# vocdoni/zk-franchise-proof-circuit

Measured on AMD Instinct MI355X. Metric: zkCensus proofs/sec (nLevels=160), higher is better.
Workload: dtype u256 (8 x u32 Montgomery, BN254 Fr/Fq)

## Files before the change

include/zkcensus.h:

```cpp
#ifndef ZKCENSUS_H
#define ZKCENSUS_H
#include <stddef.h>
#include <stdint.h>
#ifdef __cplusplus
extern "C" {
#endif

typedef struct zkc_ctx zkc_ctx;
typedef struct zkc_zkey zkc_zkey;

enum {
    ZKC_OK = 0,
    ZKC_ERR_GENERIC = 1,
    ZKC_ERR_SHORT_BUFFER = 2,
    ZKC_ERR_INVALID_WITNESS_LENGTH = 3,
    ZKC_ERR_BAD_ARG = 4,
    ZKC_ERR_FORMAT = 5,
    ZKC_ERR_HIP = 6,
    ZKC_ERR_WITNESS = 7
};
enum {
    ZKC_W_OK = 0, ZKC_W_ERR_WEIGHT = 1 , ZKC_W_ERR_SIK_ROOT = 2 ,
    ZKC_W_ERR_CENSUS_ROOT = 3 , ZKC_W_ERR_NULLIFIER = 4 , ZKC_W_ERR_LAST_SIBLING = 5 ,
    ZKC_W_ERR_INPUT_RANGE = 6 ,
    ZKC_W_ERR_SIK_LAST_SIBLING = 7
};
const char* zkc_witness_status_text(int nLevels, int32_t status);

int  zkc_ctx_create(int hip_device, zkc_ctx** out);
void zkc_ctx_destroy(zkc_ctx* ctx);
const char* zkc_last_error(const zkc_ctx* ctx);
void* zkc_ctx_stream(zkc_ctx* ctx);

int zkc_circuit_n_inputs(int nLevels);
int zkc_circuit_n_wires(int nLevels);
int zkc_circuit_nlevels_from_wasm(const void* wasm, size_t len, char sha256_hex[65]);
void zkc_sha256(const void* data, size_t len, uint8_t out[32]);

int zkc_witness(zkc_ctx* ctx, int nLevels, const void* inputs, int B, void* wtns, int32_t* status);
int zkc_inputs_from_json(const char* json, size_t len, int nLevels, void* out, char* err, size_t errlen);
int zkc_witness_dev(zkc_ctx* ctx, int nLevels, const void* d_inputs, int B, void* d_wtns, int32_t* d_status );

int  zkc_zkey_load(zkc_ctx* ctx, const void* zkey_bytes, size_t len, zkc_zkey** out);
void zkc_zkey_free(zkc_zkey* zk);
int  zkc_zkey_info(const zkc_zkey* zk, uint32_t* nVars, uint32_t* nPublic, uint32_t* domainSize);
int  zkc_zkey_pass_info(const zkc_zkey* zk, int* pass_size, int* lanes);
int  zkc_zkey_header_info(const void* zkey_bytes, size_t len, uint32_t* nVars, uint32_t* nPublic, uint32_t* domainSize);
int  zkc_zkey_sha256(const zkc_zkey* zk, uint8_t out[32]);
int  zkc_zkey_fingerprint(const void* zkey_bytes, size_t len, uint8_t out[32]);

void zkc_random_scalars(uint8_t* out, size_t n);
int zkc_prove(zkc_zkey* zk, const void* wtns, uint32_t nWitness, const uint8_t r[32], const uint8_t s[32],
              uint8_t proof[256], uint8_t* public_out);
int zkc_prove_dev(zkc_zkey* zk, const void* d_wtns, uint32_t nWitness, const uint8_t r[32], const uint8_t s[32],
                  uint8_t proof[256], uint8_t* public_out);

int zkc_prove_batch_dev(zkc_zkey* zk, const void* d_wtns, uint32_t nWitness, int B, const uint8_t* rs, uint8_t* proofs, uint8_t* publics);

int zkc_fullprove_batch_dev(zkc_zkey* zk, const void* d_inputs, int B, void* d_wtns, int32_t* d_status, const uint8_t* rs, uint8_t* proofs, uint8_t* publics);

int zkc_batch_begin(zkc_zkey* zk, int slot, const void* d_inputs, int B, void* d_wtns, int32_t* d_status, const uint8_t* rs);
int zkc_batch_finish(zkc_zkey* zk, int slot, uint8_t* proofs, uint8_t* publics);

typedef struct zkc_pool zkc_pool;
int  zkc_pool_create(const int* hip_devices, int n, zkc_pool** out);
void zkc_pool_destroy(zkc_pool* pool);
int  zkc_pool_size(const zkc_pool* pool);
zkc_ctx*  zkc_pool_ctx(zkc_pool* pool, int i);
zkc_zkey* zkc_pool_zkey(zkc_pool* pool, int i);
const char* zkc_pool_last_error(const zkc_pool* pool);
int  zkc_pool_zkey_load(zkc_pool* pool, const void* zkey_bytes, size_t len);
int  zkc_pool_fullprove_batch(zkc_pool* pool, const void* inputs, int B, const uint8_t* rs, uint8_t* proofs, uint8_t* publics, int32_t* status);

typedef struct zkc_service zkc_service;
typedef void (*zkc_done_fn)(void* user, int rc, int32_t witness_status, const char* error_text );
int  zkc_service_create(const int* hip_devices, int n, zkc_service** out);
void zkc_service_destroy(zkc_service* svc);
zkc_service* zkc_service_default(void);
const char* zkc_service_last_error(void);
int zkc_service_fullprove(zkc_service* svc, const void* zkey, size_t zkey_len, int nLevels, const void* inputs , const uint8_t* rs,
                          uint8_t proof[256], uint8_t* publics , int32_t* status, char* err, size_t errlen);
int zkc_service_prove(zkc_service* svc, const void* zkey, size_t zkey_len, const void* wtns , uint32_t nWitness, const uint8_t* rs,
                      uint8_t proof[256], uint8_t* publics, char* err, size_t errlen);
int zkc_service_fullprove_json(zkc_service* svc, const void* zkey, size_t zkey_len, const void* wasm, size_t wasm_len, const char* inputs_json, size_t inputs_len,
                               const uint8_t* rs, uint8_t proof[256], uint8_t* publics, int32_t* status, char* err, size_t errlen);
int zkc_service_submit_fullprove(zkc_service* svc, const void* zkey, size_t zkey_len, int nLevels, const void* inputs, const uint8_t* rs,
                                 uint8_t proof[256], uint8_t* publics, zkc_done_fn done, void* user);
int zkc_service_submit_prove(zkc_service* svc, const void* zkey, size_t zkey_len, const void* wtns, uint32_t nWitness, const uint8_t* rs,
                             uint8_t proof[256], uint8_t* publics, zkc_done_fn done, void* user);
int zkc_service_stats(zkc_service* svc, uint64_t out[8]);
int zkc_service_timing(zkc_service* svc, uint64_t out[8]);
int zkc_service_memory(zkc_service* svc, uint64_t out[8]);

int groth16_prover(const void* zkey_buffer, unsigned long zkey_size, const void* wtns_buffer, unsigned long wtns_size,
                   char* proof_buffer, unsigned long* proof_size, char* public_buffer, unsigned long* public_size,
                   char* error_msg, unsigned long error_msg_maxsize);

int groth16_fullprove(const void* zkey_buffer, unsigned long zkey_size, const void* wasm_buffer, unsigned long wasm_size, const char* inputs_json, unsigned long inputs_size,
                      char* proof_buffer, unsigned long* proof_size, char* public_buffer, unsigned long* public_size,
// ... 87 lines not shown
```

zk-franchise-proof-circuit_amd/__init__.py:

```python
import ctypes
from . import _native
from ._native import ZkcError
from .inputs import INPUT_KEYS, flatten_inputs, R_MOD

__all__ = ['Context', 'ProvingKey', 'DevicePool', 'ProvingService', 'groth16', 'ZkcError', 'INPUT_KEYS', 'flatten_inputs', 'R_MOD']


class Context:

    def __init__(self, device=0):
        self._lib = _native.load()
        h = ctypes.c_void_p()
        rc = self._lib.zkc_ctx_create(int(device), ctypes.byref(h))
        if rc != 0:
            raise ZkcError(rc, (self._lib.zkc_last_error(None) or b'').decode())
        self._h = h
        self.device = device
        self._keys = []

    def close(self):
        if getattr(self, '_h', None):
            for k in list(self._keys):
                k.close()
            self._lib.zkc_ctx_destroy(self._h)
            self._h = None

    def __del__(self):
        try:
            self.close()
        except Exception:
            pass

    def _check(self, rc, allow=()):
        if rc != 0 and rc not in allow:
            raise ZkcError(rc, (self._lib.zkc_last_error(self._h) or b'').decode())
        return rc

    @property
    def stream(self):
        return self._lib.zkc_ctx_stream(self._h)

    def n_wires(self, nLevels=160):
        return self._lib.zkc_circuit_n_wires(nLevels)

    def n_inputs(self, nLevels=160):
        return self._lib.zkc_circuit_n_inputs(nLevels)

    def witness(self, inputs, nLevels=160):
        flat = b''.join(x if isinstance(x, (bytes, bytearray)) else flatten_inputs(x, nLevels) for x in inputs)
        B = len(inputs)
        nw = self.n_wires(nLevels)
        out = ctypes.create_string_buffer(B * nw * 32)
        st = (ctypes.c_int32 * B)()
        self._check(self._lib.zkc_witness(self._h, nLevels, flat, B, out, st), allow=(7,))
        raw = out.raw
        return [raw[i * nw * 32:(i + 1) * nw * 32] for i in range(B)], list(st)

    def witness_dev(self, d_inputs_ptr, B, d_wtns_ptr, d_status_ptr, nLevels=160):
        self._check(self._lib.zkc_witness_dev(self._h, nLevels, d_inputs_ptr, B, d_wtns_ptr, d_status_ptr))


class ProvingKey:

    def __init__(self, ctx, zkey_bytes):
        self.ctx = ctx
        self._lib = ctx._lib
        h = ctypes.c_void_p()
        ctx._check(self._lib.zkc_zkey_load(ctx._h, zkey_bytes, len(zkey_bytes), ctypes.byref(h)))
        self._h = h
        ctx._keys.append(self)
        a, b, c = ctypes.c_uint32(), ctypes.c_uint32(), ctypes.c_uint32()
        self._lib.zkc_zkey_info(h, ctypes.byref(a), ctypes.byref(b), ctypes.byref(c))
        self.n_vars, self.n_public, self.domain_size = a.value, b.value, c.value
        ps, ln = ctypes.c_int(), ctypes.c_int()
        self._lib.zkc_zkey_pass_info(h, ctypes.byref(ps), ctypes.byref(ln))
        self.pass_size, self.lanes = ps.value, ln.value

    def close(self):
        if getattr(self, '_h', None):
            if getattr(self.ctx, '_h', None):
                self._lib.zkc_zkey_free(self._h)
            self._h = None
            if self in self.ctx._keys:
                self.ctx._keys.remove(self)

    def __del__(self):
        try:
            self.close()
        except Exception:
            pass

    @staticmethod
    def _scalar(x):
        return x if isinstance(x, (bytes, bytearray)) else int(x).to_bytes(32, 'little')

    def prove(self, wtns, r, s):
        proof = ctypes.create_string_buffer(256); pub = ctypes.create_string_buffer(32 * self.n_public)
        self.ctx._check(self._lib.zkc_prove(self._h, wtns, len(wtns) // 32, self._scalar(r), self._scalar(s), proof, pub))
        return proof.raw, pub.raw

    def prove_dev(self, d_wtns_ptr, r, s):
        proof = ctypes.create_string_buffer(256); pub = ctypes.create_string_buffer(32 * self.n_public)
        self.ctx._check(self._lib.zkc_prove_dev(self._h, d_wtns_ptr, self.n_vars, self._scalar(r), self._scalar(s), proof, pub))
        return proof.raw, pub.raw

    def prove_batch_dev(self, d_wtns_ptr, B, rs):
        proofs = ctypes.create_string_buffer(256 * B); pubs = ctypes.create_string_buffer(32 * self.n_public * B)
        self.ctx._check(self._lib.zkc_prove_batch_dev(self._h, d_wtns_ptr, self.n_vars, B, bytes(rs), proofs, pubs))
        return proofs.raw, pubs.raw

    def fullprove_batch_dev(self, d_inputs_ptr, B, d_wtns_ptr, d_status_ptr, rs):
        proofs = ctypes.create_string_buffer(256 * B); pubs = ctypes.create_string_buffer(32 * self.n_public * B)
        self.ctx._check(self._lib.zkc_fullprove_batch_dev(self._h, d_inputs_ptr, B, d_wtns_ptr, d_status_ptr, bytes(rs), proofs, pubs))
        return proofs.raw, pubs.raw

    def batch_begin(self, slot, d_inputs_ptr, B, d_wtns_ptr, d_status_ptr, rs):
        self.ctx._check(self._lib.zkc_batch_begin(self._h, slot, d_inputs_ptr, B, d_wtns_ptr, d_status_ptr, bytes(rs)))

    def batch_finish(self, slot, B):
        proofs = ctypes.create_string_buffer(256 * B); pubs = ctypes.create_string_buffer(32 * self.n_public * B)
        self.ctx._check(self._lib.zkc_batch_finish(self._h, slot, proofs, pubs))
        return proofs.raw, pubs.raw

    def debug_stage(self, d_wtns_ptr, stage):
        out = ctypes.create_string_buffer((96 if stage == 0 else 32) * self.domain_size)
        self.ctx._check(self._lib.zkc_debug_stage(self._h, d_wtns_ptr, stage, out))
        return out.raw

    def msm_debug(self, which, d_scalars_ptr, count):
# ... 114 lines not shown
```

zk-franchise-proof-circuit_amd/_native.py:

```python
import ctypes
import os

_HERE = os.path.dirname(os.path.abspath(__file__))
LIB_PATH = os.environ.get('ZKCENSUS_LIB') or os.path.join(_HERE, 'libzkcensus.so')
_lib = None


class ZkcError(RuntimeError):
    def __init__(self, code, msg):
        super().__init__('libzkcensus error %d: %s' % (code, msg))
        self.code = code


def load():
    global _lib
    if _lib is not None:
        return _lib
    if not os.path.exists(LIB_PATH):
        raise ImportError('libzkcensus.so is not built (run `python -c "import __graft_entry__ as g; g.build()"`); '
                          'there is no CPU fallback for the product path')
    try:
        import torch
    except ImportError:
        pass
    L = ctypes.CDLL(LIB_PATH)
    vp, i32p = ctypes.c_void_p, ctypes.POINTER(ctypes.c_int32)
    L.zkc_ctx_create.argtypes = [ctypes.c_int, ctypes.POINTER(vp)]
    L.zkc_ctx_destroy.argtypes = [vp]
    L.zkc_last_error.argtypes = [vp]; L.zkc_last_error.restype = ctypes.c_char_p
    L.zkc_ctx_stream.argtypes = [vp]; L.zkc_ctx_stream.restype = vp
    L.zkc_witness.argtypes = [vp, ctypes.c_int, vp, ctypes.c_int, vp, i32p]
    L.zkc_witness_dev.argtypes = [vp, ctypes.c_int, vp, ctypes.c_int, vp, vp]
    u8p, u32p = ctypes.c_char_p, ctypes.POINTER(ctypes.c_uint32)
    L.zkc_zkey_load.argtypes = [vp, ctypes.c_char_p, ctypes.c_size_t, ctypes.POINTER(vp)]
    L.zkc_zkey_free.argtypes = [vp]; L.zkc_zkey_free.restype = None
    L.zkc_zkey_info.argtypes = [vp, u32p, u32p, u32p]
    L.zkc_zkey_pass_info.argtypes = [vp, ctypes.POINTER(ctypes.c_int), ctypes.POINTER(ctypes.c_int)]
    L.zkc_witness_status_text.argtypes = [ctypes.c_int, ctypes.c_int32]; L.zkc_witness_status_text.restype = ctypes.c_char_p
    L.zkc_prove.argtypes = [vp, ctypes.c_char_p, ctypes.c_uint32, u8p, u8p, ctypes.c_char_p, ctypes.c_char_p]
    L.zkc_prove_dev.argtypes = [vp, vp, ctypes.c_uint32, u8p, u8p, ctypes.c_char_p, ctypes.c_char_p]
    L.zkc_prove_batch_dev.argtypes = [vp, vp, ctypes.c_uint32, ctypes.c_int, ctypes.c_char_p, ctypes.c_char_p, ctypes.c_char_p]
    L.zkc_fullprove_batch_dev.argtypes = [vp, vp, ctypes.c_int, vp, vp, ctypes.c_char_p, ctypes.c_char_p, ctypes.c_char_p]
    L.zkc_debug_stage.argtypes = [vp, vp, ctypes.c_int, ctypes.c_char_p]
    L.zkc_debug_early_retries.argtypes = []; L.zkc_debug_early_retries.restype = ctypes.c_ulonglong
    L.zkc_msm_debug.argtypes = [vp, ctypes.c_int, vp, ctypes.c_uint32, ctypes.c_char_p]
    L.zkc_debug_pairing_dev.argtypes = [vp, ctypes.c_char_p, ctypes.c_char_p, ctypes.c_char_p, ctypes.c_int, ctypes.c_char_p, ctypes.c_char_p, i32p, ctypes.POINTER(ctypes.c_int),
                                        ctypes.POINTER(ctypes.c_uint32), ctypes.c_size_t, ctypes.c_char_p]
    ulp = ctypes.POINTER(ctypes.c_ulong)
    L.groth16_prover.argtypes = [ctypes.c_char_p, ctypes.c_ulong, ctypes.c_char_p, ctypes.c_ulong, ctypes.c_char_p, ulp, ctypes.c_char_p, ulp, ctypes.c_char_p, ctypes.c_ulong]
    L.zkc_verify.argtypes = [ctypes.c_char_p, ctypes.c_char_p, ctypes.c_char_p]
    L.zkc_verify_bin.argtypes = [ctypes.c_char_p, ctypes.c_int, ctypes.c_char_p, ctypes.c_char_p]
    L.zkc_verify_batch.argtypes = [vp, ctypes.c_char_p, ctypes.c_int, ctypes.c_char_p, ctypes.c_char_p, ctypes.c_int, ctypes.c_char_p]
    L.zkc_verify_batch_each.argtypes = [vp, ctypes.c_char_p, ctypes.c_int, ctypes.c_char_p, ctypes.c_char_p, ctypes.c_int, ctypes.c_char_p, i32p]
    L.zkc_verify_each_stats.argtypes = [vp, ctypes.POINTER(ctypes.c_uint64)]
    L.zkc_verify_last_error.restype = ctypes.c_char_p
    L.zkc_proof_to_json.argtypes = [ctypes.c_char_p, ctypes.c_char_p, ctypes.c_int, ctypes.c_char_p, ulp, ctypes.c_char_p, ulp]
    L.zkc_proof_from_json.argtypes = [ctypes.c_char_p, ctypes.c_char_p, ctypes.c_char_p, ctypes.c_char_p, ctypes.POINTER(ctypes.c_int)]
    L.zkc_vkey_from_json.argtypes = [ctypes.c_char_p, ctypes.c_char_p, ulp, ctypes.POINTER(ctypes.c_int)]
    L.zkc_wtns_parse.argtypes = [ctypes.c_char_p, ctypes.c_ulong, ctypes.POINTER(ctypes.c_void_p), ctypes.POINTER(ctypes.c_uint32)]
    L.zkc_wtns_write.argtypes = [ctypes.c_char_p, ctypes.c_uint32, ctypes.c_char_p, ctypes.c_ulong]; L.zkc_wtns_write.restype = ctypes.c_ulong
    L.zkc_poseidon_batch.argtypes = [vp, ctypes.c_int, ctypes.c_char_p, ctypes.c_size_t, ctypes.c_char_p]
    L.zkc_smt_build.argtypes = [vp, ctypes.c_char_p, ctypes.c_char_p, ctypes.c_size_t, ctypes.c_int, ctypes.c_char_p, ctypes.c_char_p, i32p]
    L.zkc_census_inputs.argtypes = [vp, ctypes.c_size_t, ctypes.c_int, ctypes.c_char_p, ctypes.c_char_p, ctypes.c_char_p, ctypes.c_char_p, ctypes.c_char_p, ctypes.c_char_p, ctypes.c_char_p, vp, vp, ctypes.c_char_p]
    sz = ctypes.c_size_t
    L.zkc_tree_create.argtypes = [vp, ctypes.c_int, ctypes.POINTER(vp)]
    L.zkc_tree_free.argtypes = [vp]; L.zkc_tree_free.restype = None
    L.zkc_tree_add.argtypes = [vp, ctypes.c_char_p, ctypes.c_char_p, sz, i32p]
    L.zkc_tree_update.argtypes = [vp, ctypes.c_char_p, ctypes.c_char_p, sz, i32p]
    L.zkc_tree_delete.argtypes = [vp, ctypes.c_char_p, sz, i32p]
    L.zkc_tree_refs.argtypes = [vp, ctypes.POINTER(sz)]
    L.zkc_tree_snapshot.argtypes = [vp, ctypes.POINTER(vp)]
    L.zkc_tree_snapshot_count.argtypes = [vp, ctypes.POINTER(sz)]
    L.zkc_tree_gen_absence_proof.argtypes = [vp, ctypes.c_char_p, sz, ctypes.c_char_p, vp, i32p, vp, vp, i32p, i32p]
    L.zkc_tree_root.argtypes = [vp, ctypes.c_char_p]
    L.zkc_tree_size.argtypes = [vp, ctypes.POINTER(sz)]
    L.zkc_tree_get.argtypes = [vp, ctypes.c_char_p, sz, vp, i32p]
    L.zkc_tree_gen_proof.argtypes = [vp, ctypes.c_char_p, sz, ctypes.c_char_p, vp, i32p, i32p]
    L.zkc_tree_census_inputs.argtypes = [vp, vp, sz, ctypes.c_char_p, ctypes.c_char_p, ctypes.c_char_p, ctypes.c_char_p, ctypes.c_char_p, ctypes.c_char_p, vp, vp, ctypes.c_char_p, i32p]
    L.zkc_tree_stats.argtypes = [vp, ctypes.POINTER(ctypes.c_double)]
    L.zkc_smt_check_proofs.argtypes = [vp, ctypes.c_int, sz, ctypes.c_char_p, ctypes.c_char_p, ctypes.c_char_p, ctypes.c_char_p, ctypes.c_int, i32p]
    L.zkc_smt_check_absence.argtypes = [vp, ctypes.c_int, sz, ctypes.c_char_p, ctypes.c_char_p, ctypes.c_char_p, i32p, ctypes.c_char_p, ctypes.c_char_p, ctypes.c_int, i32p]
    L.zkc_smt_check_stats.argtypes = [vp, ctypes.POINTER(ctypes.c_double)]
    L.zkc_profile_enable.argtypes = [vp, ctypes.c_uint32]
    L.zkc_ntt_dev.argtypes = [vp, vp, vp, ctypes.c_int, ctypes.c_int, ctypes.c_int]
    L.zkc_g1_mul_batch_dev.argtypes = [vp, ctypes.c_char_p, vp, ctypes.c_uint32, vp]
    L.zkc_msm_g1_load_dev.argtypes = [vp, vp, ctypes.c_uint32, ctypes.POINTER(vp)]
    L.zkc_msm_g1_dev.argtypes = [vp, vp, ctypes.c_char_p]
    L.zkc_msm_g1_free.argtypes = [vp]; L.zkc_msm_g1_free.restype = None
    L.zkc_profile_read.argtypes = [vp, ctypes.c_int, ctypes.POINTER(ctypes.c_double), ctypes.POINTER(ctypes.c_uint64), ctypes.POINTER(ctypes.c_uint64)]
    L.zkc_setup_from_r1cs.argtypes = [ctypes.c_char_p, ctypes.c_uint64, ctypes.c_char_p, ctypes.c_char_p, ctypes.c_char_p, ctypes.c_size_t]
# ... 62 lines not shown
```

zk-franchise-proof-circuit_amd/csrc/zkc_api.hip:

```cpp
#include "zkc_internal.h"
#include "zkc_f29.h"
#include "zkc_kernels.h"
#include <array>
#include <cstring>
#include <ctime>
#include <map>
#include <mutex>
#include "../../include/zkc_poseidon_constants.inc"

using namespace zkc;

static constexpr int ZKC_WITNESS_WAVE_MAX_B = 128, ZKC_WITNESS_WAVE_MAX_B_ALONE = 1024;

static thread_local std::string g_create_err;

int zkc_fail(zkc_ctx* ctx, int code, const std::string& msg) {
    if (ctx) ctx->err = msg; else g_create_err = msg;
    return code;
}
hipError_t zkc_wait_event(hipEvent_t ev, unsigned spin_us) {
    if (sw::on<sw::ZKC_SPIN_WAIT>()) return hipEventSynchronize(ev);
    timespec t0; if (spin_us) clock_gettime(CLOCK_MONOTONIC, &t0);
    for (int i = 0;; i++) {
        const hipError_t e = hipEventQuery(ev);
// ... 5 lines not shown
}
hipError_t zkc_wait_stream(hipStream_t st, hipEvent_t scratch_ev) {
    const hipError_t e = hipEventRecord(scratch_ev, st);
    return e != hipSuccess ? e : zkc_wait_event(scratch_ev);
}
void zkc_ctx_lanes_destroy(zkc_ctx* ctx);
int zkc_ensure(zkc_ctx* ctx, void** p, size_t* cur, size_t need) {
    if (*cur >= need) return ZKC_OK;
    if (*p) { ZKC_HIP_CHECK(ctx, hipFree(*p)); *p = nullptr; *cur = 0; }
    ZKC_HIP_CHECK(ctx, hipMalloc(p, need));
    *cur = need;
    return ZKC_OK;
}

void zkc_verify_ws_trim(zkc_ctx* ctx, size_t keep_bytes) {
    size_t total = 0; for (size_t b : ctx->vws_sz) total += b;
    if (total <= keep_bytes && keep_bytes) return;
    for (int i = 0; i < zkc_ctx::VWS_N; i++) { if (ctx->vws[i]) (void)hipFree(ctx->vws[i]); ctx->vws[i] = nullptr; ctx->vws_sz[i] = 0; }
}

static hipEvent_t prof_event(zkc_ctx* ctx) {
    if (!ctx->prof.free_events.empty()) { hipEvent_t e = ctx->prof.free_events.back(); ctx->prof.free_events.pop_back(); return e; }
    hipEvent_t e = nullptr; (void)hipEventCreate(&e); return e;
}
zkc_prof_scope::zkc_prof_scope(zkc_ctx* c, int category, uint64_t alg_bytes, hipStream_t stream) : ctx(c), cat(category), st(stream ? stream : (c ? c->stream : nullptr)) {
    on = c && ((c->prof.mask >> category) & 1u);
    if (!on) return;
    a = prof_event(c); b = prof_event(c);
    c->prof.bytes[cat] += alg_bytes; c->prof.launches[cat] += 1;
    (void)hipEventRecord(a, st);
}
zkc_prof_scope::~zkc_prof_scope() {
    if (!on) return;
    (void)hipEventRecord(b, st);
    ctx->prof.pending.push_back({a, b, cat});
}
extern "C" int zkc_profile_enable(zkc_ctx* ctx, uint32_t mask) {
    if (!ctx) return ZKC_ERR_BAD_ARG;
    ZKC_LOCK(ctx);
    ZKC_HIP_CHECK(ctx, hipSetDevice(ctx->device));
    (void)hipStreamSynchronize(ctx->stream);
    for (auto& r : ctx->prof.pending) { ctx->prof.free_events.push_back(r.a); ctx->prof.free_events.push_back(r.b); }
    ctx->prof.pending.clear();
    for (int i = 0; i < ZKC_PROF_NCAT; i++) { ctx->prof.ms[i] = 0; ctx->prof.launches[i] = 0; ctx->prof.bytes[i] = 0; }
    if (!ctx->d_prof_entries && hipMalloc((void**)&ctx->d_prof_entries, 8) != hipSuccess) ctx->d_prof_entries = nullptr;
    if (ctx->d_prof_entries) (void)hipMemset(ctx->d_prof_entries, 0, 8);
    ctx->prof.mask = mask;
    return ZKC_OK;
}
extern "C" int zkc_profile_read(zkc_ctx* ctx, int cat, double* total_ms, uint64_t* launches, uint64_t* alg_bytes) {
    if (!ctx || cat < 0 || cat >= ZKC_PROF_NCAT) return ZKC_ERR_BAD_ARG;
    ZKC_LOCK(ctx);
    ZKC_HIP_CHECK(ctx, hipSetDevice(ctx->device));
    ZKC_HIP_CHECK(ctx, hipStreamSynchronize(ctx->stream)); ZKC_HIP_CHECK(ctx, hipStreamSynchronize(ctx->stream2)); ZKC_HIP_CHECK(ctx, hipStreamSynchronize(ctx->fin_stream));
    for (auto& r : ctx->prof.pending) {
        float ms = 0; (void)hipEventElapsedTime(&ms, r.a, r.b); ctx->prof.ms[r.cat] += ms;
        ctx->prof.free_events.push_back(r.a); ctx->prof.free_events.push_back(r.b);
    }
    ctx->prof.pending.clear();
    if (cat == ZKC_PROF_MSM_G1_STREAMED && ctx->d_prof_entries) {
        unsigned long long v = 0; (void)hipMemcpyAsync(&v, ctx->d_prof_entries, 8, hipMemcpyDeviceToHost, ctx->stream); (void)hipStreamSynchronize(ctx->stream); ctx->prof.launches[cat] = v;
    }
    if (total_ms) *total_ms = ctx->prof.ms[cat]; if (launches) *launches = ctx->prof.launches[cat]; if (alg_bytes) *alg_bytes = ctx->prof.bytes[cat];
    return ZKC_OK;
}

extern "C" int zkc_poseidon_batch(zkc_ctx* ctx, int n_inputs, const void* inputs, size_t B, void* out) {
    if (!ctx || !inputs || !out || n_inputs < 2 || n_inputs > 4 || B == 0) return zkc_fail(ctx, ZKC_ERR_BAD_ARG, "zkc_poseidon_batch: bad argument");
    ZKC_LOCK(ctx);
    ZKC_HIP_CHECK(ctx, hipSetDevice(ctx->device));
    int rc;
    if ((rc = zkc_ensure(ctx, &ctx->d_scratch_in, &ctx->scratch_in_sz, B * n_inputs * 32))) return rc;
    if ((rc = zkc_ensure(ctx, &ctx->d_scratch_out, &ctx->scratch_out_sz, B * 32))) return rc;
    ZKC_HIP_CHECK(ctx, hipMemcpyAsync(ctx->d_scratch_in, inputs, B * n_inputs * 32, hipMemcpyHostToDevice, ctx->stream));
    hipLaunchKernelGGL(zkc_poseidon_batch_kernel, dim3((unsigned)((B + 63) / 64)), dim3(64), 0, ctx->stream, ctx->ptab, (const uint32_t*)ctx->d_scratch_in,
                       (uint32_t*)ctx->d_scratch_out, n_inputs, B);
    ZKC_HIP_CHECK(ctx, hipGetLastError());
    ZKC_HIP_CHECK(ctx, hipMemcpyAsync(out, ctx->d_scratch_out, B * 32, hipMemcpyDeviceToHost, ctx->stream));
    ZKC_HIP_CHECK(ctx, hipStreamSynchronize(ctx->stream));
    return ZKC_OK;
}

__global__ void zkc_status_combine(const int32_t* __restrict__ s3, int32_t* __restrict__ s, int B) {
    int b = blockIdx.x * blockDim.x + threadIdx.x;
    if (b >= B) return;
    int m = s3[3 * b + 2], c = s3[3 * b + 0], k = s3[3 * b + 1], r = 0;
    if (m == ZKC_W_ERR_INPUT_RANGE) r = m;
    else if (m == ZKC_W_ERR_WEIGHT) r = m;
    else if (k) r = k; else if (c) r = c; else r = m;
    s[b] = r;
}

template <size_t N>
static void conv_consts(std::vector<Fr>& out, const unsigned long long (&src)[N][4]) {
    for (size_t i = 0; i < N; i++) {
        uint32_t s[8];
        for (int k = 0; k < 4; k++) { s[2 * k] = (uint32_t)src[i][k]; s[2 * k + 1] = (uint32_t)(src[i][k] >> 32); }
        out.push_back(fp_from_std<FrParams>(s));
    }
}


extern "C" int zkc_ctx_create(int device, zkc_ctx** out) {
    if (!out) return zkc_fail(nullptr, ZKC_ERR_BAD_ARG, "out == NULL");
    int ndev = 0;
    if (hipGetDeviceCount(&ndev) != hipSuccess || ndev <= 0)
        return zkc_fail(nullptr, ZKC_ERR_HIP, "no HIP device: libzkcensus has no CPU path (the CPU restatement lives in oracle/ and is test-only)");
    if (device < 0 || device >= ndev) return zkc_fail(nullptr, ZKC_ERR_BAD_ARG, "bad device ordinal");
    zkc_ctx* ctx = new zkc_ctx();
    ctx->device = device;
    auto fail = [&](hipError_t e, const char* what) { g_create_err = std::string(what) + ": " + hipGetErrorString(e); delete ctx; return (int)ZKC_ERR_HIP; };
    hipError_t e;
    if ((e = hipSetDevice(device)) != hipSuccess) return fail(e, "hipSetDevice");
    { if (sw::on<sw::ZKC_DEVICE_BLOCKING_SYNC>() && hipSetDeviceFlags(hipDeviceScheduleBlockingSync) != hipSuccess) (void)hipGetLastError(); }
    if ((e = hipStreamCreateWithFlags(&ctx->stream, hipStreamNonBlocking)) != hipSuccess) return fail(e, "hipStreamCreate");
    if ((e = hipStreamCreateWithFlags(&ctx->stream2, hipStreamNonBlocking)) != hipSuccess) return fail(e, "hipStreamCreate(2)");
    if ((e = hipStreamCreateWithFlags(&ctx->fin_stream, hipStreamNonBlocking)) != hipSuccess) return fail(e, "hipStreamCreate(fin)");
    std::vector<Fr> all; size_t off[12]; int k = 0;
    off[k++] = all.size(); conv_consts(all, ZKC_POSEIDON_C3); off[k++] = all.size(); conv_consts(all, ZKC_POSEIDON_S3);
    off[k++] = all.size(); conv_consts(all, ZKC_POSEIDON_M3); off[k++] = all.size(); conv_consts(all, ZKC_POSEIDON_P3);
    off[k++] = all.size(); conv_consts(all, ZKC_POSEIDON_C4); off[k++] = all.size(); conv_consts(all, ZKC_POSEIDON_S4);
    off[k++] = all.size(); conv_consts(all, ZKC_POSEIDON_M4); off[k++] = all.size(); conv_consts(all, ZKC_POSEIDON_P4);
    off[k++] = all.size(); conv_consts(all, ZKC_POSEIDON_C5); off[k++] = all.size(); conv_consts(all, ZKC_POSEIDON_S5);
    off[k++] = all.size(); conv_consts(all, ZKC_POSEIDON_M5); off[k++] = all.size(); conv_consts(all, ZKC_POSEIDON_P5);
    if ((e = hipMalloc(&ctx->d_ptab_mem, all.size() * sizeof(Fr))) != hipSuccess) return fail(e, "hipMalloc(poseidon)");
    if ((e = hipMemcpy(ctx->d_ptab_mem, all.data(), all.size() * sizeof(Fr), hipMemcpyHostToDevice)) != hipSuccess) return fail(e, "hipMemcpy(poseidon)");
    const Fr* base = (const Fr*)ctx->d_ptab_mem;
    {
        std::vector<uint32_t> l29(all.size() * 12, 0);
        for (size_t i = 0; i < all.size(); i++) { uint32_t t9[9]; f29_from_fp_shl5(t9, all[i].v); f29_mul<FrParams>(&l29[12 * i], t9, F29K<FrParams>::one.l); }
        if ((e = hipMalloc(&ctx->d_ptab29_mem, l29.size() * 4)) != hipSuccess) return fail(e, "hipMalloc(poseidon29)");
        if ((e = hipMemcpy(ctx->d_ptab29_mem, l29.data(), l29.size() * 4, hipMemcpyHostToDevice)) != hipSuccess) return fail(e, "hipMemcpy(poseidon29)");
        ctx->ptab.base = base; ctx->ptab.base29 = (const uint32_t*)ctx->d_ptab29_mem;
        std::vector<uint32_t> k29; size_t koff[2];
        for (int t = 3; t <= 4; t++) {
            koff[t - 3] = k29.size();
            const int RP = t == 3 ? 57 : 56; const size_t oC = off[(t - 3) * 4 + 0], oS = off[(t - 3) * 4 + 1];
            for (int r = 0; r < RP; r++) for (int k = 0; k < t; k++) {
                const size_t si = oS + (size_t)(2 * t - 1) * r + (k ? t + k - 1 : 0), ci = oC + 5 * t + r;
                const Fr prod = all[si] * all[ci];
                uint32_t t9[9], o9[12] = {0}; f29_from_fp_shl5(t9, prod.v); f29_mul<FrParams>(o9, t9, F29K<FrParams>::one.l); f29_reduce_small<FrParams>(o9);
                k29.insert(k29.end(), o9, o9 + 12);
            }
        }
        if ((e = hipMalloc(&ctx->d_pk29_mem, k29.size() * 4)) != hipSuccess) return fail(e, "hipMalloc(poseidon K29)");
        if ((e = hipMemcpy(ctx->d_pk29_mem, k29.data(), k29.size() * 4, hipMemcpyHostToDevice)) != hipSuccess) return fail(e, "hipMemcpy(poseidon K29)");
        for (int t = 3; t <= 4; t++) ctx->ptab.K29[t] = (const uint32_t*)ctx->d_pk29_mem + koff[t - 3];
    }
    for (int t = 3; t <= 5; t++) {
        ctx->ptab.C[t] = base + off[(t - 3) * 4 + 0]; ctx->ptab.S[t] = base + off[(t - 3) * 4 + 1];
        ctx->ptab.M[t] = base + off[(t - 3) * 4 + 2]; ctx->ptab.P[t] = base + off[(t - 3) * 4 + 3];
    }
    *out = ctx;
    return ZKC_OK;
}
extern "C" void zkc_ctx_destroy(zkc_ctx* ctx) {
    if (!ctx) return;
    (void)hipSetDevice(ctx->device);
    if (ctx->stream) (void)hipStreamSynchronize(ctx->stream);
    for (auto& r : ctx->prof.pending) { (void)hipEventDestroy(r.a); (void)hipEventDestroy(r.b); }
    for (auto e : ctx->prof.free_events) (void)hipEventDestroy(e);
    for (auto& kv : ctx->tmpl) (void)hipFree(kv.second);
    for (auto& kv : ctx->ntt_tw) { if (kv.second.fwd) (void)hipFree(kv.second.fwd); if (kv.second.inv) (void)hipFree(kv.second.inv); if (kv.second.ninv) (void)hipFree(kv.second.ninv); }
    if (ctx->d_ptab_mem) (void)hipFree(ctx->d_ptab_mem);
    if (ctx->d_ptab29_mem) (void)hipFree(ctx->d_ptab29_mem);
    if (ctx->d_pk29_mem) (void)hipFree(ctx->d_pk29_mem);
    if (ctx->d_scratch_in) (void)hipFree(ctx->d_scratch_in);
    if (ctx->d_scratch_out) (void)hipFree(ctx->d_scratch_out);
    if (ctx->d_status3) (void)hipFree(ctx->d_status3);
    if (ctx->d_status) (void)hipFree(ctx->d_status);
    if (ctx->d_prof_entries) (void)hipFree(ctx->d_prof_entries);
    for (int k = 0; k < 2; k++) {
        if (ctx->chk_h[k]) (void)hipHostFree(ctx->chk_h[k]);
        if (ctx->chk_d[k]) (void)hipFree(ctx->chk_d[k]);
        if (ctx->chk_ev[k]) (void)hipEventDestroy(ctx->chk_ev[k]);
    }
    zkc_verify_ws_trim(ctx, 0);
    if (ctx->ev_vws_up) (void)hipEventDestroy(ctx->ev_vws_up);
    if (ctx->ev_vws_lines) (void)hipEventDestroy(ctx->ev_vws_lines);
    for (auto& ls : ctx->lane_streams) for (hipStream_t q : {ls.st, ls.st2, ls.fin, ls.red}) if (q) (void)hipStreamSynchronize(q);
    zkc_ctx_lanes_destroy(ctx);
    if (ctx->ev_acc_chain) (void)hipEventDestroy(ctx->ev_acc_chain);
    if (ctx->stream2) (void)hipStreamDestroy(ctx->stream2);
    if (ctx->fin_stream) (void)hipStreamDestroy(ctx->fin_stream);
    if (ctx->stream) (void)hipStreamDestroy(ctx->stream);
    delete ctx;
}
int zkc_lane_streams(zkc_ctx* ctx, int l, bool with_red, zkc_ctx::LaneStreams* out) {
    if (!ctx || l < 0 || l >= 4 || !out) return ZKC_ERR_BAD_ARG;
    static std::mutex mu; static std::map<int, std::array<zkc_ctx::LaneStreams, 4>> by_device;
    std::lock_guard<std::mutex> g(mu);
    zkc_ctx::LaneStreams& ls = by_device[ctx->device][l];
    for (hipStream_t* q : {&ls.st, &ls.st2, &ls.fin}) if (!*q) ZKC_HIP_CHECK(ctx, hipStreamCreateWithFlags(q, hipStreamNonBlocking));
    if (with_red && !ls.red) ZKC_HIP_CHECK(ctx, hipStreamCreateWithFlags(&ls.red, hipStreamNonBlocking));
    ctx->lane_streams[l] = ls; *out = ls; return ZKC_OK;
}
extern "C" const char* zkc_last_error(const zkc_ctx* ctx) { return ctx ? ctx->err.c_str() : g_create_err.c_str(); }
extern "C" void* zkc_ctx_stream(zkc_ctx* ctx) { return ctx ? (void*)ctx->stream : nullptr; }
extern "C" int zkc_circuit_n_inputs(int nLevels) { return nLevels < 3 ? 0 : WitnessLayout::make(nLevels).nInputs; }
extern "C" int zkc_circuit_n_wires(int nLevels) { return nLevels < 3 ? 0 : WitnessLayout::make(nLevels).nWires; }

static int get_template(zkc_ctx* ctx, const WitnessLayout& L, uint32_t** out) {
    auto it = ctx->tmpl.find(L.nL);
    if (it != ctx->tmpl.end()) { *out = it->second; return ZKC_OK; }
    uint32_t *d_t = nullptr, *d_in = nullptr; int32_t* d_st = nullptr;
    const int rc = [&]() -> int {
        ZKC_HIP_CHECK(ctx, hipMalloc(&d_t, (size_t)L.nWires * 32));
        ZKC_HIP_CHECK(ctx, hipMalloc(&d_in, (size_t)L.nInputs * 32));
        ZKC_HIP_CHECK(ctx, hipMalloc(&d_st, 3 * sizeof(int32_t)));
        ZKC_HIP_CHECK(ctx, hipMemsetAsync(d_t, 0, (size_t)L.nWires * 32, ctx->stream));
        ZKC_HIP_CHECK(ctx, hipMemsetAsync(d_in, 0, (size_t)L.nInputs * 32, ctx->stream));
        hipLaunchKernelGGL(zkc_witness_chains_wave, dim3(3), dim3(64), 0, ctx->stream, L, ctx->ptab, d_in, d_t, d_st, 1, 1);
        hipLaunchKernelGGL(zkc_witness_tostd, dim3((L.nWires + 255) / 256), dim3(256), 0, ctx->stream, d_t, (size_t)L.nWires);
        ZKC_HIP_CHECK(ctx, hipGetLastError());
        ZKC_HIP_CHECK(ctx, hipStreamSynchronize(ctx->stream));
        return ZKC_OK;
    }();
    if (d_in) (void)hipFree(d_in);
    if (d_st) (void)hipFree(d_st);
    if (rc) { if (d_t) (void)hipFree(d_t); return rc; }
    ctx->tmpl[L.nL] = d_t; *out = d_t;
    return ZKC_OK;
}

uint32_t* zkc_get_template(zkc_ctx* ctx, int nLevels) {
    uint32_t* t = nullptr; WitnessLayout L = WitnessLayout::make(nLevels);
    return get_template(ctx, L, &t) == ZKC_OK ? t : nullptr;
}

static int witness_dev3(zkc_ctx* ctx, const WitnessLayout& L, const void* d_inputs, int B, void* d_wtns, int32_t* d_status3, bool alone, hipStream_t st = nullptr) {
    if (!st) st = ctx->stream;
    uint32_t* tmpl; int rc = get_template(ctx, L, &tmpl); if (rc) return rc;
    const size_t total = (size_t)L.nWires * 2 * (size_t)B;
    int fill_blocks = (int)std::min<size_t>((total + 255) / 256, 256 * 16);
    zkc_prof_scope _ps(ctx, ZKC_PROF_WITNESS, (uint64_t)B * ((uint64_t)L.nWires + L.nInputs) * 32, st);
    hipLaunchKernelGGL(zkc_witness_fill, dim3(fill_blocks), dim3(256), 0, st, (const uint4*)tmpl, (uint4*)d_wtns, L.nWires, B);
    ZKC_HIP_CHECK(ctx, hipGetLastError());
    if (B <= (alone ? ZKC_WITNESS_WAVE_MAX_B_ALONE : ZKC_WITNESS_WAVE_MAX_B))
        hipLaunchKernelGGL(zkc_witness_chains_wave, dim3(3 * B), dim3(64), 0, st, L, ctx->ptab, (const uint32_t*)d_inputs, (uint32_t*)d_wtns, d_status3, B, 0);
    else
        hipLaunchKernelGGL(zkc_witness_chains, dim3((3 * B + 63) / 64), dim3(64), 0, st, L, ctx->ptab, (const uint32_t*)d_inputs, (uint32_t*)d_wtns, d_status3, B, 0);
    {
        const size_t nw = (size_t)L.nWires * (size_t)B;
        hipLaunchKernelGGL(zkc_witness_tostd, dim3((unsigned)std::min<size_t>((nw + 255) / 256, 256 * 64)), dim3(256), 0, st, (uint32_t*)d_wtns, nw);
    }
    ZKC_HIP_CHECK(ctx, hipGetLastError());
// ... 43 lines not shown
```

zk-franchise-proof-circuit_amd/csrc/zkc_internal.h:

```cpp
#pragma once
#include <hip/hip_runtime.h>
#include <string>
#include <vector>
#include <map>
#include <mutex>
#include "../../include/zkcensus.h"
#include "zkc_device.h"
#include "zkc_switches.h"

#define ZKC_LOCK(ctx) std::lock_guard<std::recursive_mutex> _zkc_guard((ctx)->mu)
#define ZKC_HIP_CHECK(ctx, call)                                                                            \
    do { hipError_t _e = (call); if (_e != hipSuccess) {                                                     \
        return zkc_fail((ctx), ZKC_ERR_HIP, std::string(#call) + ": " + hipGetErrorString(_e)); } } while (0)

enum { ZKC_PROF_WITNESS = 0, ZKC_PROF_MATVEC = 1, ZKC_PROF_NTT = 2, ZKC_PROF_MSM_SORT = 3, ZKC_PROF_MSM_ACC_G1 = 4, ZKC_PROF_MSM_ACC_G2 = 5,
       ZKC_PROF_MSM_REDUCE = 6, ZKC_PROF_MSM_G1_STREAMED = 7 , ZKC_PROF_NCAT = 8 };
struct zkc_prof {
    uint32_t mask = 0;
    struct Rec { hipEvent_t a, b; int cat; };
    std::vector<Rec> pending; std::vector<hipEvent_t> free_events;
    double ms[ZKC_PROF_NCAT] = {0}; uint64_t launches[ZKC_PROF_NCAT] = {0}; uint64_t bytes[ZKC_PROF_NCAT] = {0};
};
struct zkc_ctx {
    std::recursive_mutex mu;
    int device = 0;
    hipStream_t stream = nullptr;
    hipStream_t stream2 = nullptr;
    hipStream_t fin_stream = nullptr;
    struct LaneStreams { hipStream_t st = nullptr, st2 = nullptr, fin = nullptr, red = nullptr; } lane_streams[4];
    struct zkc_lane* lanes = nullptr;
    hipEvent_t ev_acc_chain = nullptr; bool acc_chain_armed = false;
    std::string err;
    zkc::PoseidonTable ptab{};
    void* d_ptab_mem = nullptr;
    void* d_ptab29_mem = nullptr;
    void* d_pk29_mem = nullptr;
    std::map<int, uint32_t*> tmpl;
    struct TwiddleSet { uint32_t *fwd = nullptr, *inv = nullptr; void* ninv = nullptr; };
    std::map<int, TwiddleSet> ntt_tw;
    void* d_scratch_in = nullptr; size_t scratch_in_sz = 0;
    void* d_scratch_out = nullptr; size_t scratch_out_sz = 0;
    int32_t* d_status3 = nullptr; size_t status3_n = 0;
    int32_t* d_status = nullptr; size_t status_n = 0;
    enum { VWS_PTS = 0, VWS_RHO, VWS_IDX, VWS_GS, VWS_FOLD_TMP, VWS_FOLD_OUT, VWS_Q, VWS_LINES, VWS_TREE_A, VWS_TREE_B, VWS_BAD,
           VWS_FLAGS, VWS_SUM_TREE, VWS_TREE_ALL, VWS_NODES , VWS_N };
    void* vws[VWS_N] = {nullptr}; size_t vws_sz[VWS_N] = {0};
    uint64_t each_stats[4] = {0, 0, 0, 0};
    hipEvent_t ev_vws_up = nullptr, ev_vws_lines = nullptr;
    void* chk_h[2] = {nullptr, nullptr}; void* chk_d[2] = {nullptr, nullptr}; size_t chk_sz = 0; hipEvent_t chk_ev[2] = {nullptr, nullptr};
    double chk_ms[3] = {0, 0, 0};
    double r1cs_ms[3] = {0, 0, 0};
    zkc_prof prof;
    unsigned long long* d_prof_entries = nullptr;
};

int zkc_fail(zkc_ctx* ctx, int code, const std::string& msg);
hipError_t zkc_wait_event(hipEvent_t ev, unsigned spin_us = 0);
hipError_t zkc_wait_stream(hipStream_t st, hipEvent_t scratch_ev);
int zkc_ensure(zkc_ctx* ctx, void** p, size_t* cur, size_t need);
inline int zkc_vws(zkc_ctx* ctx, int which, size_t need, void** out) { const int rc = zkc_ensure(ctx, &ctx->vws[which], &ctx->vws_sz[which], need); *out = ctx->vws[which]; return rc; }
void zkc_verify_ws_trim(zkc_ctx* ctx, size_t keep_bytes);
struct zkc_prof_scope {
    zkc_ctx* ctx; int cat; hipEvent_t a = nullptr, b = nullptr; bool on; hipStream_t st;
    zkc_prof_scope(zkc_ctx* c, int category, uint64_t alg_bytes, hipStream_t stream = nullptr);
    ~zkc_prof_scope();
};
```

zk-franchise-proof-circuit_amd/csrc/zkc_pairing_dev.hip:

```cpp
#include <algorithm>
#include <cstdio>
#include <cstdlib>
#include <ctime>
#include <vector>
#include "zkc_prover.h"
#include "zkc_pairing.h"
#include "zkc_pairing_dev.h"

namespace zkc {
using namespace zkc::pairing;

struct MillerConsts { Fq2 twist_b, psi_x, psi_y, psi2_x, psi2_y; Fq half; uint64_t pos, neg; uint64_t t_lo, t_hi; };

__device__ __forceinline__ void store_line(Fq2* __restrict__ lines, uint32_t N, uint32_t step, uint32_t i, const Fq2 l[3]) {
    Fq2* o = lines + ((size_t)step * N + i) * 3; o[0] = l[0]; o[1] = l[1]; o[2] = l[2];
}
__device__ __forceinline__ bool g2_member(const G2Affine& q, const MillerConsts& C) {
    bool ok = fp_sqr(q.y) == fp_sqr(q.x) * q.x + C.twist_b;
    if (ok) {
        G2XYZZ acc = G2XYZZ::from_affine(q);
        for (int b = 125; b >= 0; b--) { acc = xyzz_dbl(acc); if (((b < 64 ? C.t_lo >> b : C.t_hi >> (b - 64)) & 1)) acc = xyzz_add_affine(acc, q); }
        ok = !acc.is_inf() && acc.X == conj2(q.x) * C.psi_x * acc.ZZ && acc.Y == conj2(q.y) * C.psi_y * acc.ZZZ;
    }
    return ok;
// ... 32 lines not shown
        if ((C.pos >> b) & 1) { line_add(R, q.x, q.y, l); store_line(lines, N, step++, i, l); }
        else if ((C.neg >> b) & 1) { line_add(R, q.x, nqy, l); store_line(lines, N, step++, i, l); }
    }
    line_add(R, conj2(q.x) * C.psi_x, conj2(q.y) * C.psi_y, l); store_line(lines, N, step++, i, l);
    line_add(R, q.x * C.psi2_x, fp_neg(q.y * C.psi2_y), l); store_line(lines, N, step++, i, l);
}
__device__ __forceinline__ void line_at(const Fq2* __restrict__ raw, const G1XYZZ& p, Fq2 out[3]) {
    if (p.is_inf()) { out[0] = Fq2::one(); out[1] = out[2] = Fq2::zero(); return; }
    out[0] = scale2(raw[0], fp_neg(p.Y * p.ZZ)); out[1] = scale2(raw[1], p.X * p.ZZZ); out[2] = scale2(raw[2], p.ZZ * p.ZZZ);
}
__global__ void __launch_bounds__(64)
zkc_line_pairs(const Fq2* __restrict__ lines, const G1XYZZ* __restrict__ P, uint32_t N, uint32_t nlines, Fq12* __restrict__ out) {
    const uint32_t half = (N + 1) / 2, gid = blockIdx.x * blockDim.x + threadIdx.x;
    if (gid >= nlines * half) return;
    const uint32_t s = gid / half, t = gid - s * half;
    const Fq2* a = lines + ((size_t)s * N + 2 * t) * 3;
    Fq2 l0[3], l1[3];
    line_at(a, P[2 * t], l0);
    if (2 * t + 1 < N) { line_at(a + 3, P[2 * t + 1], l1); out[(size_t)s * half + t] = mul_034_by_034(l0, l1); }
    else out[(size_t)s * half + t] = dense_of_034(l0);
}
__global__ void __launch_bounds__(64)
zkc_fq12_tree(const Fq12* __restrict__ in, uint32_t n, uint32_t nlines, Fq12* __restrict__ out) {
    const uint32_t half = (n + 1) / 2, gid = blockIdx.x * blockDim.x + threadIdx.x;
    if (gid >= nlines * half) return;
    const uint32_t s = gid / half, t = gid - s * half;
    const Fq12* a = in + (size_t)s * n + 2 * t;
    out[(size_t)s * half + t] = (2 * t + 1 < n) ? a[0] * a[1] : a[0];
}
__global__ void __launch_bounds__(64)
zkc_g1_sum_tree(const G1XYZZ* __restrict__ in, uint32_t n, G1XYZZ* __restrict__ out) {
    const uint32_t t = blockIdx.x * blockDim.x + threadIdx.x;
    if (t >= (n + 1) / 2) return;
    out[t] = (2 * t + 1 < n) ? xyzz_add(in[2 * t], in[2 * t + 1]) : in[2 * t];
}
__global__ void __launch_bounds__(64)
zkc_fq12_node(const Fq12* __restrict__ level, uint32_t m, uint32_t t, uint32_t nlines, Fq12* __restrict__ out) {
    const uint32_t s = blockIdx.x * blockDim.x + threadIdx.x;
    if (s < nlines && t < m) out[s] = level[(size_t)s * m + t];
}

static MillerConsts miller_consts() {
    const Consts& K = consts(); const AteLoop& L = ate_loop();
    MillerConsts C; C.twist_b = K.twist_b; C.psi_x = K.psi_x; C.psi_y = K.psi_y; C.psi2_x = K.psi2_x; C.psi2_y = K.psi2_y; C.half = K.half; C.pos = C.neg = 0;
    for (int b = 0; b < 64; b++) { if (L.digit[b] > 0) C.pos |= 1ull << b; else if (L.digit[b] < 0) C.neg |= 1ull << b; }
    C.t_lo = 0xf83e9682e87cfd46ull; C.t_hi = 0x6f4d8248eeb859fbull;
    return C;
}
static int dev_fail(zkc_ctx* ctx, hipError_t e, const char* what) { ctx->err = std::string(what) + ": " + hipGetErrorString(e); (void)hipGetLastError(); return ZKC_ERR_HIP; }

uint32_t verify_chunk() { return (uint32_t)sw::value<sw::ZKC_VERIFY_CHUNK>(16384); }
static uint32_t n_lines(const MillerConsts& C) { return 66 + (uint32_t)__builtin_popcountll(C.pos | C.neg); }
uint32_t verify_n_lines() { return n_lines(miller_consts()); }
void miller_join(zkc_ctx* ctx) { (void)hipStreamSynchronize(ctx->stream2); (void)hipStreamSynchronize(ctx->fin_stream); }

int miller_membership_begin(zkc_ctx* ctx, const G2Affine* h_Q, uint32_t N) {
    const MillerConsts C = miller_consts();
    const uint32_t cap = std::min(N, verify_chunk());
    void* q; int rc;
    if ((rc = zkc_vws(ctx, zkc_ctx::VWS_Q, (size_t)N * sizeof(G2Affine), &q))) return rc;
    G2Affine* d_Q = (G2Affine*)q;
    if ((rc = zkc_vws(ctx, zkc_ctx::VWS_BAD, sizeof(int), &q))) return rc;
    int* d_bad = (int*)q;
    if ((rc = zkc_vws(ctx, zkc_ctx::VWS_LINES, (size_t)n_lines(C) * cap * 3 * sizeof(Fq2), &q))) return rc;
    Fq2* d_lines = (Fq2*)q;
    hipError_t e;
    if (!ctx->ev_vws_up && (e = hipEventCreateWithFlags(&ctx->ev_vws_up, hipEventDisableTiming)) != hipSuccess) return dev_fail(ctx, e, "miller_membership_begin: hipEventCreate");
    if (!ctx->ev_vws_lines && (e = hipEventCreateWithFlags(&ctx->ev_vws_lines, hipEventDisableTiming)) != hipSuccess) return dev_fail(ctx, e, "miller_membership_begin: hipEventCreate");
    if ((e = hipMemcpyAsync(d_Q, h_Q, (size_t)N * sizeof(G2Affine), hipMemcpyHostToDevice, ctx->stream2)) != hipSuccess ||
        (e = hipMemsetAsync(d_bad, 0, sizeof(int), ctx->stream2)) != hipSuccess ||
        (e = hipEventRecord(ctx->ev_vws_up, ctx->stream2)) != hipSuccess ||
        (e = hipStreamWaitEvent(ctx->fin_stream, ctx->ev_vws_up, 0)) != hipSuccess ||
        (e = hipStreamWaitEvent(ctx->stream, ctx->ev_vws_up, 0)) != hipSuccess) { miller_join(ctx); return dev_fail(ctx, e, "miller_membership_begin: upload"); }
    hipLaunchKernelGGL(zkc_g2_membership, dim3((N + 63) / 64), dim3(64), 0, ctx->stream2, d_Q, N, C, d_bad);
    hipLaunchKernelGGL(zkc_miller_lines, dim3((cap + 63) / 64), dim3(64), 0, ctx->fin_stream, d_Q, cap, C, d_lines);
    if ((e = hipGetLastError()) != hipSuccess || (e = hipEventRecord(ctx->ev_vws_lines, ctx->fin_stream)) != hipSuccess) { miller_join(ctx); return dev_fail(ctx, e, "miller_membership_begin: launch"); }
    return ZKC_OK;
}
int miller_product_dev(zkc_ctx* ctx, const G1XYZZ* d_P, uint32_t N, Fq12* product, int* bad, std::vector<Fq12>* tops) {
    const MillerConsts C = miller_consts();
    const uint32_t nlines = n_lines(C), CHUNK = verify_chunk();
    const uint32_t cap = std::min(N, CHUNK), hcap = (cap + 1) / 2;
    const bool vtrace = sw::on<sw::ZKC_VERIFY_TRACE>();
    auto vnow = [] { timespec ts; clock_gettime(CLOCK_MONOTONIC, &ts); return ts.tv_sec * 1e3 + ts.tv_nsec * 1e-6; };
    const double mt0 = vnow(); double mt_chunks = 0;
    std::vector<Fq12> step(nlines), acc(nlines, one12());
    const int rc = [&]() -> int {
        const G2Affine* d_Q = (const G2Affine*)ctx->vws[zkc_ctx::VWS_Q];
        Fq2* d_lines = (Fq2*)ctx->vws[zkc_ctx::VWS_LINES];
        Fq12 *d_a, *d_b; void* q; int r;
        if ((r = zkc_vws(ctx, zkc_ctx::VWS_TREE_A, (size_t)nlines * hcap * sizeof(Fq12), &q))) return r; d_a = (Fq12*)q;
        if ((r = zkc_vws(ctx, zkc_ctx::VWS_TREE_B, (size_t)nlines * ((hcap + 1) / 2) * sizeof(Fq12), &q))) return r; d_b = (Fq12*)q;
        hipError_t e;
        for (uint32_t lo = 0; lo < N; lo += CHUNK) {
            const uint32_t n = std::min(CHUNK, N - lo);
            if ((e = hipStreamWaitEvent(ctx->stream, ctx->ev_vws_lines, 0)) != hipSuccess) return dev_fail(ctx, e, "miller_product_dev: event");
            uint32_t m = (n + 1) / 2;
            hipLaunchKernelGGL(zkc_line_pairs, dim3((nlines * m + 63) / 64), dim3(64), 0, ctx->stream, d_lines, d_P + lo, n, nlines, d_a);
            if (lo + CHUNK < N) {
                const uint32_t lo2 = lo + CHUNK, n2 = std::min(CHUNK, N - lo2);
                if ((e = hipEventRecord(ctx->ev_vws_up, ctx->stream)) != hipSuccess || (e = hipStreamWaitEvent(ctx->fin_stream, ctx->ev_vws_up, 0)) != hipSuccess) return dev_fail(ctx, e, "miller_product_dev: event");
                hipLaunchKernelGGL(zkc_miller_lines, dim3((n2 + 63) / 64), dim3(64), 0, ctx->fin_stream, d_Q + lo2, n2, C, d_lines);
                if ((e = hipEventRecord(ctx->ev_vws_lines, ctx->fin_stream)) != hipSuccess) return dev_fail(ctx, e, "miller_product_dev: event");
            }
            Fq12 *src = d_a, *dst = d_b;
            while (m > 1) {
                const uint32_t h = (m + 1) / 2;
                hipLaunchKernelGGL(zkc_fq12_tree, dim3((nlines * h + 63) / 64), dim3(64), 0, ctx->stream, src, m, nlines, dst);
                std::swap(src, dst); m = h;
            }
            if ((e = hipGetLastError()) != hipSuccess) return dev_fail(ctx, e, "miller_product_dev: launch");
            if ((e = hipMemcpyAsync(step.data(), src, (size_t)nlines * sizeof(Fq12), hipMemcpyDeviceToHost, ctx->stream)) != hipSuccess ||
// ... 93 lines not shown
```

zk-franchise-proof-circuit_amd/csrc/zkc_prove.hip:

```cpp
#include "zkc_prover.h"
#include "zkc_fixedbase.h"
#include "zkc_hostparse.h"
#include "zkc_kernels.h"
#include <cstring>
#include <ctime>
#include <cstdio>
#include <algorithm>
#include <atomic>

using namespace zkc;

static void matvec_launch(zkc_zkey* zk, zkc_lane& L, const uint32_t* d_wtns0, int nb, hipStream_t mv) {
    const uint32_t n = zk->n, nv = zk->nVars;
    const bool units = zk->n_unit_coeffs > 0 && nv <= 3 * (size_t)n && sw::on<sw::ZKC_MATVEC_UNITS>();
    if (units) hipLaunchKernelGGL(zkc_wtns_mont, dim3((nv + 255) / 256, nb), dim3(256), 0, mv, (const Fr*)d_wtns0, (size_t)nv, L.d_t, 3 * (size_t)n, nv);
    hipLaunchKernelGGL(zkc_matvec_jds, dim3((2 * n + 63 * zk->nlong + 255) / 256, nb), dim3(256), 0, mv, zk->d_perm, zk->d_rowlen, zk->d_jdptr, zk->d_col, zk->d_val,
                       (const Fr*)d_wtns0, (size_t)nv, L.d_abc, (int)n, zk->nlong, units ? (const Fr*)L.d_t : (const Fr*)nullptr, 3 * (size_t)n);
    hipLaunchKernelGGL(zkc_pointwise_mul, dim3((n + 255) / 256, nb), dim3(256), 0, mv, L.d_abc, (int)n);
}
static constexpr uint32_t MATVEC_LONG = 16;

namespace {
uint32_t rd32(const uint8_t* p) { uint32_t v; memcpy(&v, p, 4); return v; }
uint64_t rd64(const uint8_t* p) { uint64_t v; memcpy(&v, p, 8); return v; }
G1Affine rd_g1(const uint8_t* p) { G1Affine a; memcpy(a.x.v, p, 32); memcpy(a.y.v, p + 32, 32); return a; }
G2Affine rd_g2(const uint8_t* p) { G2Affine a; memcpy(a.x.c0.v, p, 32); memcpy(a.x.c1.v, p + 32, 32); memcpy(a.y.c0.v, p + 64, 32); memcpy(a.y.c1.v, p + 96, 32); return a; }
Fr fr_root_of_unity(int logn) {
    uint32_t e[8]; for (int i = 0; i < 8; i++) e[i] = FrParams::p[i]; e[0] -= 1;
    for (int i = 0; i < 8; i++) e[i] = (e[i] >> 28) | (i < 7 ? e[i + 1] << 4 : 0);
    Fr g = fp_from_u32<FrParams>(5), w = Fr::one();
    for (int i = 255; i >= 0; i--) { w = w * w; if ((e[i >> 5] >> (i & 31)) & 1) w = w * g; }
    for (int i = 28; i > logn; i--) w = w * w;
    return w;
}
template <class T> int dmalloc(zkc_ctx* ctx, T** p, size_t count) { ZKC_HIP_CHECK(ctx, hipMalloc((void**)p, count * sizeof(T))); return ZKC_OK; }
void g1_to_std(uint8_t* out, const G1Affine& a) { uint32_t s[8]; fp_to_std<FqParams>(s, a.x); memcpy(out, s, 32); fp_to_std<FqParams>(s, a.y); memcpy(out + 32, s, 32); }
void g2_to_std(uint8_t* out, const G2Affine& a) {
    uint32_t s[8]; fp_to_std<FqParams>(s, a.x.c0); memcpy(out, s, 32); fp_to_std<FqParams>(s, a.x.c1); memcpy(out + 32, s, 32);
    fp_to_std<FqParams>(s, a.y.c0); memcpy(out + 64, s, 32); fp_to_std<FqParams>(s, a.y.c1); memcpy(out + 96, s, 32);
}
}

uint32_t* zkc_get_template(zkc_ctx* ctx, int nLevels);
int zkc_lane_streams(zkc_ctx* ctx, int l, bool with_red, zkc_ctx::LaneStreams* out);

extern "C" __global__ void __launch_bounds__(64)
zkc_fold_check(WitnessLayout L, const uint32_t* __restrict__ wtns, const uint32_t* __restrict__ tmpl, uint32_t* __restrict__ flags, int B) {
    const int n = L.n, g = blockIdx.x, tree = blockIdx.y, b = blockIdx.z;
    const int blk = tree == 0 ? L.off_census : L.off_sikver;
    int start, end;
    if (g < n - 1) {
        const int nctrl = (g == n - 3) + (g > 0 && g < n - 2) + 1;
        start = blk + L.lvl_off(g) + nctrl; end = blk + (g + 1 < n - 1 ? L.lvl_off(g + 1) : L.lvl_off(n - 1));
    } else { start = blk + L.off_n2bold; end = start + 253 + 127 + 133; }
    const uint4* w = reinterpret_cast<const uint4*>(wtns + (size_t)b * L.nWires * 8) + 2 * (size_t)start;
    const uint4* t = reinterpret_cast<const uint4*>(tmpl) + 2 * (size_t)start;
    uint32_t diff = 0;
    for (int i = threadIdx.x; i < 2 * (end - start); i += 64) { uint4 x = w[i], y = t[i]; diff |= (x.x ^ y.x) | (x.y ^ y.y) | (x.z ^ y.z) | (x.w ^ y.w); }
    const unsigned long long any = __ballot(diff != 0);
    if (threadIdx.x == 0) flags[((size_t)b * 2 + tree) * n + g] = any ? 1u : 0u;
}

extern "C" __global__ void __launch_bounds__(64)
zkc_input_depths(const uint32_t* __restrict__ inputs, int nInputs, int n, uint32_t* __restrict__ out) {
    const int b = blockIdx.x, tree = blockIdx.y;
    const uint32_t* sib = inputs + ((size_t)b * nInputs + 12 + (size_t)tree * n) * 8;
    int d = 0;
    for (int i = threadIdx.x; i < n; i += 64) {
        const uint4* q = reinterpret_cast<const uint4*>(sib + 8 * (size_t)i); const uint4 x = q[0], y = q[1];
        if (x.x | x.y | x.z | x.w | y.x | y.y | y.z | y.w) d = i + 1;
    }
    for (int m = 32; m >= 1; m >>= 1) { const int o = __shfl_xor(d, m, 64); d = o > d ? o : d; }
    if (threadIdx.x == 0) out[2 * b + tree] = (uint32_t)d;
}

extern "C" void zkc_zkey_free(zkc_zkey* zk) {
    if (!zk) return;
    ZKC_LOCK(zk->ctx);
    (void)hipSetDevice(zk->ctx->device);
    (void)hipStreamSynchronize(zk->ctx->stream);
    void* ptrs[] = {zk->d_perm, zk->d_rowlen, zk->d_jdptr, zk->d_col, zk->d_val, zk->d_tw_fwd, zk->d_tw_inv, zk->d_tw_fwd29, zk->d_tw_inv29, zk->d_coset, zk->d_coset_br, zk->d_g1, zk->d_g2, zk->d_g2_29, zk->d_g2_29_lone, zk->d_g2_29_deep,
                    zk->d_tblDelta1, zk->d_tblAlpha1, zk->d_tblBeta1, zk->d_tblDelta2, zk->d_fb4, zk->d_fb4g2, zk->d_depths};
    for (void* p : ptrs) if (p) (void)hipFree(p);
    for (auto& kv : zk->fold.vmaps) if (kv.second.d) (void)hipFree(kv.second.d);
    for (void* q : {(void*)zk->fold.d_foldA, (void*)zk->fold.d_foldB1, (void*)zk->fold.d_foldC, (void*)zk->fold.d_foldB2}) if (q) (void)hipFree(q);
    if (zk->h_depths) (void)hipHostFree(zk->h_depths);
    for (auto& c : zk->call) { for (void* q : {(void*)c.d_rs, (void*)c.d_proofs, (void*)c.d_flags, (void*)c.d_status3}) if (q) (void)hipFree(q); if (c.h_flags) (void)hipHostFree(c.h_flags); if (c.h_out) (void)hipHostFree(c.h_out); if (c.h_rs) (void)hipHostFree(c.h_rs); if (c.h_xyzz) (void)hipHostFree(c.h_xyzz); if (c.h_early) (void)hipHostFree(c.h_early); if (c.d_xyzz) (void)hipFree(c.d_xyzz); for (hipEvent_t e : c.ev_done) if (e) (void)hipEventDestroy(e); for (hipEvent_t e : c.ev_chunk) (void)hipEventDestroy(e); }
    if (zk->ctx->lanes) for (int l = 0; l < zk->nlanes; l++) for (hipStream_t q : {zk->ctx->lanes[l].st, zk->ctx->lanes[l].st2, zk->ctx->lanes[l].fin, zk->ctx->lanes[l].red}) if (q) (void)hipStreamSynchronize(q);
    delete zk;
}

static size_t dev_free_bytes() { size_t f = 0, t = 0; if (hipMemGetInfo(&f, &t) != hipSuccess) { (void)hipGetLastError(); return 0; } return f; }
static int fold_prepare(zkc_zkey* zk);
static int fb4_prepare(zkc_zkey* zk);
struct LaneNeed { size_t abc, p, fin, bs, e1, b1, e2, b2; int j1, j2; };
static LaneNeed lane_need(const zkc_zkey* zk, int inflight) {
    const uint32_t n = zk->n, nv = zk->nVars; const int NWS = msm_nw(zk->c_sec), NWB = msm_nw(zk->c_h);
    const size_t per_proof_entries = (size_t)NWS * 3 * nv + (size_t)NWB * n;
    const size_t per_proof_buckets = 3 * (size_t)msm_half(std::max(zk->c_sec, zk->c_deep)) + msm_half(zk->c_h);
    LaneNeed nd; nd.abc = 3 * (size_t)n * inflight; nd.p = 8 * (size_t)n * inflight; nd.fin = finalize_scratch_bytes(inflight); nd.bs = 2 * 2 * 8 * (size_t)nv;
    nd.e1 = per_proof_entries * inflight; nd.b1 = per_proof_buckets * inflight; nd.j1 = 4 * inflight;
    nd.e2 = (size_t)NWS * nv * inflight; nd.b2 = (size_t)msm_half(std::max(zk->c_sec, zk->c_deep)) * inflight; nd.j2 = inflight;
    return nd;
}
static bool lane_holds(const zkc_lane& L, const LaneNeed& nd) {
    return L.cap_abc >= nd.abc && L.cap_p >= nd.p && L.cap_fin >= nd.fin && L.cap_bs >= nd.bs && L.w1.max_entries >= nd.e1 && L.w1.max_buckets >= nd.b1 && L.w1.max_jobs >= nd.j1 &&
           L.w2.max_entries >= nd.e2 && L.w2.max_buckets >= nd.b2 && L.w2.max_jobs >= nd.j2;
}
static void lane_release(zkc_lane& L) {
    for (void** q : {(void**)&L.d_abc, (void**)&L.d_t, (void**)&L.d_p, &L.d_fin, (void**)&L.d_bs}) if (*q) { (void)hipFree(*q); *q = nullptr; }
    msm_work_free(L.w1); msm_work_free(L.w2);
    L.cap_abc = L.cap_p = L.cap_fin = L.cap_bs = 0; L.bytes = 0;
}
static zkc_lane* ctx_lanes(zkc_ctx* ctx) { if (!ctx->lanes) ctx->lanes = new zkc_lane[MAX_LANES]; return ctx->lanes; }
static size_t ctx_work_bytes(const zkc_ctx* ctx) { size_t t = 0; if (ctx->lanes) for (int l = 0; l < MAX_LANES; l++) t += ctx->lanes[l].bytes; return t; }
void zkc_ctx_lanes_destroy(zkc_ctx* ctx) {
    if (!ctx->lanes) return;
    for (int l = 0; l < MAX_LANES; l++) {
        zkc_lane& L = ctx->lanes[l];
        lane_release(L);
        for (hipEvent_t e : {L.ev_msm, L.ev_msm2, L.ev_sorted, L.ev_ntt, L.ev_mv, L.ev_acc, L.ev_fin[0], L.ev_fin[1], L.ev_red}) if (e) (void)hipEventDestroy(e);
    }
    delete[] ctx->lanes; ctx->lanes = nullptr;
}
static int lane_init(zkc_ctx* ctx, int l) {
    zkc_lane& L = ctx_lanes(ctx)[l];
    if (L.made) return ZKC_OK;
    zkc_ctx::LaneStreams ls; int rc = zkc_lane_streams(ctx, l, sw::on<sw::ZKC_REDUCE_STREAM>(), &ls); if (rc) return rc;
    L.st = ls.st; L.st2 = ls.st2; L.fin = ls.fin; L.red = ls.red;
    for (hipEvent_t* e : {&L.ev_msm, &L.ev_msm2, &L.ev_sorted, &L.ev_ntt, &L.ev_mv, &L.ev_acc, &L.ev_fin[0], &L.ev_fin[1], &L.ev_red}) if (!*e) ZKC_HIP_CHECK(ctx, hipEventCreateWithFlags(e, hipEventDisableTiming));
    L.made = true; return ZKC_OK;
}
struct LaneSt { hipStream_t st, st2, fin, red; };
static LaneSt lane_st(const zkc_zkey* zk, const zkc_lane& L) { hipStream_t c = zk->ctx->stream; return zk->serial_streams ? LaneSt{c, c, c, c} : LaneSt{L.st, L.st2, L.fin, L.red}; }
static int lane_ensure(zkc_zkey* zk, int l, int inflight) {
    zkc_ctx* ctx = zk->ctx; int rc;
    if ((rc = lane_init(ctx, l))) return rc;
    zkc_lane& L = ctx->lanes[l];
    inflight = std::max(1, std::min(inflight, zk->max_inflight));
    if (lane_holds(L, lane_need(zk, inflight))) return ZKC_OK;
    inflight = std::min(inflight <= 4 ? 4 : zk->max_inflight, zk->max_inflight);
    LaneNeed nd = lane_need(zk, inflight);
    nd.abc = std::max(nd.abc, L.cap_abc); nd.p = std::max(nd.p, L.cap_p); nd.fin = std::max(nd.fin, L.cap_fin); nd.bs = std::max(nd.bs, L.cap_bs);
    nd.e1 = std::max(nd.e1, L.w1.max_entries); nd.b1 = std::max(nd.b1, L.w1.max_buckets); nd.j1 = std::max(nd.j1, L.w1.max_jobs);
    nd.e2 = std::max(nd.e2, L.w2.max_entries); nd.b2 = std::max(nd.b2, L.w2.max_buckets); nd.j2 = std::max(nd.j2, L.w2.max_jobs);
    for (hipStream_t q : {L.st, L.st2, L.fin, L.red}) if (q) ZKC_HIP_CHECK(ctx, hipStreamSynchronize(q));
    ZKC_HIP_CHECK(ctx, hipStreamSynchronize(ctx->stream));
    lane_release(L);
    const size_t free_before = dev_free_bytes();
    const auto fail_at = sw::given<sw::ZKC_TEST_FAIL_ALLOC>();
    rc = (fail_at && inflight >= *fail_at) ? zkc_fail(ctx, ZKC_ERR_HIP, "lanes_ensure: allocation failure injected by ZKC_TEST_FAIL_ALLOC") : ZKC_OK;
    if (!rc) rc = dmalloc(ctx, &L.d_abc, nd.abc);
    if (!rc) rc = dmalloc(ctx, &L.d_t, nd.abc);
    if (!rc) rc = dmalloc(ctx, &L.d_p, nd.p);
    if (!rc && hipMalloc(&L.d_fin, nd.fin) != hipSuccess) rc = zkc_fail(ctx, ZKC_ERR_HIP, "lanes_ensure: hipMalloc failed (blinding scratch)");
    if (!rc) rc = dmalloc(ctx, &L.d_bs, nd.bs);
    if (!rc) rc = msm_work_alloc(ctx, L.w1, nd.e1, nd.b1, nd.j1, false);
    if (!rc) rc = msm_work_alloc(ctx, L.w2, nd.e2, nd.b2, nd.j2, true);
    if (rc) { (void)hipGetLastError(); lane_release(L); return rc; }
    L.cap_abc = nd.abc; L.cap_p = nd.p; L.cap_fin = nd.fin; L.cap_bs = nd.bs;
    { const size_t f = dev_free_bytes(); L.bytes = free_before > f ? free_before - f : 0; }
    return ZKC_OK;
}
static int lanes_ensure(zkc_zkey* zk, int inflight, int first = 0, int count = -1) {
    if (count < 0) count = zk->nlanes - first;
    for (int l = first; l < first + count && l < zk->nlanes; l++) { const int rc = lane_ensure(zk, l, inflight); if (rc) return rc; }
    return ZKC_OK;
}
extern "C" int zkc_zkey_load(zkc_ctx* ctx, const void* zkey_bytes, size_t len, zkc_zkey** out) { return zkc::zkey_load_opts(ctx, zkey_bytes, len, 0, 0, out); }
size_t zkc::zkey_device_bytes(const zkc_zkey* zk, size_t* tables, size_t* work) {
    if (!zk) return 0;
    const size_t w = ctx_work_bytes(zk->ctx);
    if (tables) *tables = zk->bytes_tables; if (work) *work = w;
    return zk->bytes_tables + w;
}
int zkc::zkey_load_opts(zkc_ctx* ctx, const void* zkey_bytes, size_t len, int opt_lanes, int opt_inflight, zkc_zkey** out) {
    if (!ctx || !zkey_bytes || !out) return zkc_fail(ctx, ZKC_ERR_BAD_ARG, "zkc_zkey_load: bad argument");
    ZKC_LOCK(ctx);
    ZKC_HIP_CHECK(ctx, hipSetDevice(ctx->device));
    const size_t free_at_entry = dev_free_bytes(), work_at_entry = ctx_work_bytes(ctx);
    const uint8_t* buf = (const uint8_t*)zkey_bytes;
    parse::BinSections bs; parse::ZkeyHeader zh; std::string perr;
    if (!parse::binfile_sections(buf, len, "zkey", 1, bs, perr) || !parse::zkey_check(bs, zh, perr)) return zkc_fail(ctx, ZKC_ERR_FORMAT, perr);
    const uint8_t* const* sec = bs.sec;
    const uint8_t* h = sec[2];
    zkc_zkey* zk = new zkc_zkey(); zk->ctx = ctx;
    zk->nVars = zh.nVars; zk->nPub = zh.nPub; zk->n = zh.n; zk->logn = zh.logn; zk->nCoeffs = zh.nCoeffs;
    parse::sha256(buf, len, zk->sha256); parse::zkey_fingerprint(buf, len, bs, zk->fingerprint);
    const uint32_t n = zk->n, nv = zk->nVars, np = zk->nPub, nc = nv - np - 1;
    zk->alpha1 = rd_g1(h + 84); zk->beta1 = rd_g1(h + 148); zk->beta2 = rd_g2(h + 212); zk->gamma2 = rd_g2(h + 340);
// ... 71 lines not shown
      zk->c_deep = (zk->nLevels >= 0 && (nv >= (1u << 16) || dt == 2) && zk->c_sec < cd && dt != 0) ? cd : 0; }
    zk->c_h = std::max(zk->c_h, std::max(zk->c_sec, zk->c_deep));
    const int NWB = msm_nw(zk->c_h);
    zk->offA = 0; zk->offB1 = NWS * nv; zk->offC = 2 * NWS * nv; zk->offH = 2 * NWS * nv + NWS * nc;
    const int NWD = zk->c_deep ? msm_nw(zk->c_deep) : 0;
    zk->offA_deep = zk->offH + NWB * n; zk->offB1_deep = zk->offA_deep + NWD * nv; zk->offC_deep = zk->offB1_deep + NWD * nv;
    const size_t g1_points = (size_t)NWS * (2 * (size_t)nv + nc) + (size_t)NWB * n + (size_t)NWD * (2 * (size_t)nv + nc);
    if (g1_points >= (1ull << 31)) return bail(zkc_fail(ctx, ZKC_ERR_FORMAT, "zkey too large for 31-bit point indices"));
    if ((rc = dmalloc(ctx, &zk->d_g1, g1_points)) || (rc = dmalloc(ctx, &zk->d_g2, (size_t)NWS * nv))) return bail(rc);
    ZKC_UP(zk->d_g1 + zk->offA, sec[5], 64ull * nv); ZKC_UP(zk->d_g1 + zk->offB1, sec[6], 64ull * nv);
    ZKC_UP(zk->d_g1 + zk->offC, sec[8], 64ull * nc); ZKC_UP(zk->d_g1 + zk->offH, sec[9], 64ull * n);
    ZKC_UP(zk->d_g2, sec[7], 128ull * nv);
    if ((rc = msm_precompute_g1(ctx, nv, zk->d_g1 + zk->offA, zk->c_sec)) || (rc = msm_precompute_g1(ctx, nv, zk->d_g1 + zk->offB1, zk->c_sec)) ||
        (rc = msm_precompute_g1(ctx, nc, zk->d_g1 + zk->offC, zk->c_sec)) || (rc = msm_precompute_g1(ctx, n, zk->d_g1 + zk->offH, zk->c_h)) ||
        (rc = msm_precompute_g2(ctx, nv, zk->d_g2, zk->c_sec))) return bail(rc);
    if ((rc = dmalloc(ctx, &zk->d_g2_29, 60 * (size_t)NWS * nv)) || (rc = msm_g2_table29(ctx, zk->d_g2, zk->d_g2_29, (size_t)NWS * nv))) return bail(rc);
    if (zk->c_deep) {
        ZKC_UP(zk->d_g1 + zk->offA_deep, sec[5], 64ull * nv); ZKC_UP(zk->d_g1 + zk->offB1_deep, sec[6], 64ull * nv); ZKC_UP(zk->d_g1 + zk->offC_deep, sec[8], 64ull * nc);
        if ((rc = msm_precompute_g1(ctx, nv, zk->d_g1 + zk->offA_deep, zk->c_deep)) || (rc = msm_precompute_g1(ctx, nv, zk->d_g1 + zk->offB1_deep, zk->c_deep)) ||
            (rc = msm_precompute_g1(ctx, nc, zk->d_g1 + zk->offC_deep, zk->c_deep))) return bail(rc);
        G2Affine* tmp = nullptr;
        if ((rc = dmalloc(ctx, &tmp, (size_t)NWD * nv))) return bail(rc);
        hipError_t e2 = hipMemcpyAsync(tmp, zk->d_g2, 128ull * nv, hipMemcpyDeviceToDevice, ctx->stream);
        if (e2 == hipSuccess) rc = msm_precompute_g2(ctx, nv, tmp, zk->c_deep);
        if (e2 == hipSuccess && !rc) rc = dmalloc(ctx, &zk->d_g2_29_deep, 60 * (size_t)NWD * nv);
        if (e2 == hipSuccess && !rc) rc = msm_g2_table29(ctx, tmp, zk->d_g2_29_deep, (size_t)NWD * nv);
        if (e2 == hipSuccess && !rc) e2 = hipStreamSynchronize(ctx->stream);
        (void)hipFree(tmp);
        if (rc) return bail(rc);
        if (e2 != hipSuccess) return bail(zkc_fail(ctx, ZKC_ERR_HIP, std::string("second section tables: ") + hipGetErrorString(e2)));
    }
    {
        if (sw::on<sw::ZKC_G2_LONE_TABLE>() && (zk->nLevels >= 0 || nv < (1u << 16))) {
            constexpr int NWL = msm_nw(MSM_C_G2_LONE);
            G2Affine* tmp = nullptr;
            if ((rc = dmalloc(ctx, &tmp, (size_t)NWL * nv))) return bail(rc);
            hipError_t e2 = hipMemcpyAsync(tmp, zk->d_g2, 128ull * nv, hipMemcpyDeviceToDevice, ctx->stream);
            if (e2 == hipSuccess) rc = msm_precompute_g2(ctx, nv, tmp, MSM_C_G2_LONE);
            if (e2 == hipSuccess && !rc) rc = dmalloc(ctx, &zk->d_g2_29_lone, 60 * (size_t)NWL * nv);
            if (e2 == hipSuccess && !rc) rc = msm_g2_table29(ctx, tmp, zk->d_g2_29_lone, (size_t)NWL * nv);
            if (e2 == hipSuccess && !rc) e2 = hipStreamSynchronize(ctx->stream);
            (void)hipFree(tmp);
            if (rc) return bail(rc);
            if (e2 != hipSuccess) return bail(zkc_fail(ctx, ZKC_ERR_HIP, std::string("lone-proof G2 table: ") + hipGetErrorString(e2)));
        }
    }
    const auto e_inf = sw::given<sw::ZKC_INFLIGHT>();
    zk->max_inflight = opt_inflight > 0 ? std::min(opt_inflight, MSM_MAX_JOBS / 4) : e_inf ? (int)*e_inf : zk->nLevels >= 0 ? 64 : 96;
    {
        const size_t per_proof_entries = (size_t)NWS * 3 * nv + (size_t)NWB * n, census_pass = 96ull * (22ull * 3 * 82754 + 15ull * 131072);
        const int fit = (int)std::max<size_t>(1, census_pass / std::max<size_t>(per_proof_entries, 1));
        zk->max_inflight = std::min(zk->max_inflight, fit);
    }
    { const auto e_l = sw::given<sw::ZKC_LANES>(); zk->nlanes = opt_lanes > 0 ? std::min(opt_lanes, (int)MAX_LANES) : e_l ? (int)*e_l : zk->nLevels >= 0 ? (int)MAX_LANES : 1; }
    zk->serial_streams = sw::on<sw::ZKC_SERIAL_STREAMS>();
    if ((rc = lanes_ensure(zk, 1, 0, 1))) return bail(rc);
    {
        FixedBase<Fq> td(zk->delta1), ta(zk->alpha1), tb(zk->beta1); FixedBase<Fq2> t2(zk->delta2);
        if ((rc = dmalloc(ctx, &zk->d_tblDelta1, td.tab.size())) || (rc = dmalloc(ctx, &zk->d_tblAlpha1, ta.tab.size())) ||
            (rc = dmalloc(ctx, &zk->d_tblBeta1, tb.tab.size())) || (rc = dmalloc(ctx, &zk->d_tblDelta2, t2.tab.size()))) return bail(rc);
        ZKC_UP(zk->d_tblDelta1, td.tab.data(), td.tab.size() * sizeof(G1Affine)); ZKC_UP(zk->d_tblAlpha1, ta.tab.data(), ta.tab.size() * sizeof(G1Affine));
        ZKC_UP(zk->d_tblBeta1, tb.tab.data(), tb.tab.size() * sizeof(G1Affine)); ZKC_UP(zk->d_tblDelta2, t2.tab.data(), t2.tab.size() * sizeof(G2Affine));
    }
    ZKC_HIP_BAIL(hipStreamSynchronize(ctx->stream));
    if (zk->nLevels >= 0 && (rc = fold_prepare(zk))) return bail(rc);
    if ((rc = fb4_prepare(zk))) return bail(rc);
    { const size_t f = dev_free_bytes(), grown = ctx_work_bytes(ctx) > work_at_entry ? ctx_work_bytes(ctx) - work_at_entry : 0; zk->bytes_tables = free_at_entry > f + grown ? free_at_entry - f - grown : 0; }
    *out = zk;
    return ZKC_OK;
#undef ZKC_UP
#undef ZKC_HIP_BAIL
}

int zkc::prove_reserve(zkc_zkey* zk, int inflight) {
    if (!zk) return ZKC_ERR_BAD_ARG;
    ZKC_LOCK(zk->ctx);
    ZKC_HIP_CHECK(zk->ctx, hipSetDevice(zk->ctx->device));
    return lanes_ensure(zk, inflight);
}
extern "C" int zkc_zkey_pass_info(const zkc_zkey* zk, int* pass_size, int* lanes) {
    if (!zk) return ZKC_ERR_BAD_ARG;
    if (pass_size) *pass_size = zk->max_inflight; if (lanes) *lanes = zk->nlanes;
    return ZKC_OK;
}
extern "C" int zkc_zkey_info(const zkc_zkey* zk, uint32_t* nVars, uint32_t* nPublic, uint32_t* domainSize) {
    if (!zk) return ZKC_ERR_BAD_ARG;
    if (nVars) *nVars = zk->nVars; if (nPublic) *nPublic = zk->nPub; if (domainSize) *domainSize = zk->n;
    return ZKC_OK;
}

static std::vector<std::pair<int, int>> fold_group_ranges(const WitnessLayout& L, int tree) {
    std::vector<std::pair<int, int>> r; const int n = L.n, blk = tree == 0 ? L.off_census : L.off_sikver;
    for (int g = 0; g < n - 1; g++) {
        const int nctrl = (g == n - 3) + (g > 0 && g < n - 2) + 1;
        r.push_back({blk + L.lvl_off(g) + nctrl, blk + (g + 1 < n - 1 ? L.lvl_off(g + 1) : L.lvl_off(n - 1))});
    }
    r.push_back({blk + L.off_n2bold, blk + L.off_n2bold + 253 + 127 + 133});
    return r;
}
template <class X> static void suffix_sums(std::vector<X>& suf, const X* g, int n) {
    suf.assign(n, X::inf());
    for (int D = n - 2; D >= 0; D--) suf[D] = xyzz_add(suf[D + 1], g[D]);
}
template <class PT> static int fold_upload(zkc_ctx* ctx, PT** d, const std::vector<PT>& b, const std::vector<PT>* suf) {
    std::vector<PT> t; t.push_back(b[0]); t.insert(t.end(), suf[0].begin(), suf[0].end()); t.insert(t.end(), suf[1].begin(), suf[1].end());
    ZKC_HIP_CHECK(ctx, hipMalloc((void**)d, t.size() * sizeof(PT)));
    ZKC_HIP_CHECK(ctx, hipMemcpy(*d, t.data(), t.size() * sizeof(PT), hipMemcpyHostToDevice));
    return ZKC_OK;
// ... 118 lines not shown
    if (!zk || !d_wtns || !host_out) return ZKC_ERR_BAD_ARG;
    zkc_ctx* ctx = zk->ctx; const uint32_t n = zk->n;
    ZKC_LOCK(ctx);
    ZKC_HIP_CHECK(ctx, hipSetDevice(ctx->device)); ZKC_HIP_CHECK(ctx, hipStreamSynchronize(ctx->stream));
    { int rc0 = lanes_ensure(zk, 1, 0, 1); if (rc0) return rc0; }
    zkc_lane& L0 = ctx->lanes[0]; const hipStream_t st0 = lane_st(zk, L0).st;
    if (stage == 0) {
        matvec_launch(zk, L0, (const uint32_t*)d_wtns, 1, st0);
        ZKC_HIP_CHECK(ctx, hipGetLastError());
        ZKC_HIP_CHECK(ctx, hipMemcpyAsync(host_out, L0.d_abc, 96ull * n, hipMemcpyDeviceToHost, st0));
    } else {
        int rc = h_evals_dev(zk, L0, st0, (const uint32_t*)d_wtns, 1); if (rc) return rc;
        ZKC_HIP_CHECK(ctx, hipMemcpyAsync(host_out, L0.d_p, 32ull * n, hipMemcpyDeviceToHost, st0));
    }
    ZKC_HIP_CHECK(ctx, hipStreamSynchronize(st0));
    return ZKC_OK;
}

extern "C" int zkc_msm_debug(zkc_zkey* zk, int which, const void* d_scalars, uint32_t count, void* host_out) {
    if (!zk || !d_scalars || !host_out || which < 0 || which > 4) return ZKC_ERR_BAD_ARG;
    zkc_ctx* ctx = zk->ctx;
    ZKC_LOCK(ctx);
    ZKC_HIP_CHECK(ctx, hipSetDevice(ctx->device)); ZKC_HIP_CHECK(ctx, hipStreamSynchronize(ctx->stream));
    { int rc0 = lanes_ensure(zk, 1, 0, 1); if (rc0) return rc0; }
    zkc_lane& L0 = ctx->lanes[0]; const hipStream_t st_l0 = lane_st(zk, L0).st;
    const uint32_t full = which == 3 ? zk->nVars - zk->nPub - 1 : which == 4 ? zk->n : zk->nVars;
    if (count != full) return zkc_fail(ctx, ZKC_ERR_BAD_ARG, "zkc_msm_debug: count must equal the section size");
    static thread_local MsmJobList jl; jl.clear(256, 1024, which == 2 ? (uint32_t)MSM_MAX_VW_PER_JOB : (uint32_t)MSM_MAX_VW_G1);
    const uint32_t offs[5] = {zk->offA, zk->offB1, 0, zk->offC, zk->offH};
    jl.add((const uint32_t*)d_scalars, nullptr, count, offs[which], full, 0, which == 4 ? zk->c_h : zk->c_sec);
    int rc = which == 2 ? msm_pass_g2(zk, L0.w2, jl, 0, true, st_l0) : msm_pass_g1(zk, L0.w1, jl, 0, true, st_l0); if (rc) return rc;
    ZKC_HIP_CHECK(ctx, hipStreamSynchronize(st_l0));
    if (which == 2) g2_to_std((uint8_t*)host_out, xyzz_to_affine(*(G2XYZZ*)L0.w2.h_results));
    else g1_to_std((uint8_t*)host_out, xyzz_to_affine(*(G1XYZZ*)L0.w1.h_results));
    return ZKC_OK;
}

int zkc_witness_chunk_async(zkc_ctx* ctx, int nLevels, const void* d_inputs, int B, void* d_wtns, int32_t* d_status3, int32_t* d_status, hipStream_t st);
int zkc::prove_batch_begin(zkc_zkey* zk, int cs, const void* d_wtns, uint32_t nWitness, int B, const uint8_t* rs, bool want_publics, const void* d_inputs, int32_t* d_status,
                           int lane0, hipEvent_t wait_first, const uint8_t* host_depths, bool no_early) {
    if (!zk || !d_wtns || !rs || B <= 0 || cs < 0 || cs >= CALL_SLOTS || lane0 >= zk->nlanes) return zkc_fail(zk ? zk->ctx : nullptr, ZKC_ERR_BAD_ARG, "zkc_prove_batch_dev: bad argument");
    zkc_ctx* ctx = zk->ctx;
    ZKC_LOCK(ctx);
    if (nWitness != zk->nVars) return zkc_fail(ctx, ZKC_ERR_INVALID_WITNESS_LENGTH, "Invalid witness length. Circuit: " + std::to_string(zk->nVars) + ", witness: " + std::to_string(nWitness));
    for (int b = 0; b < 2 * B; b++) { uint32_t t[8]; memcpy(t, rs + 32 * (size_t)b, 32); if (!fp_std_lt_p<FrParams>(t)) return zkc_fail(ctx, ZKC_ERR_BAD_ARG, "r or s >= field order"); }
    ZKC_HIP_CHECK(ctx, hipSetDevice(ctx->device));
    const uint32_t nv = zk->nVars, np = zk->nPub, nc = nv - np - 1, n = zk->n;
    const bool can_fold = zk->nLevels >= 0;
    WitnessLayout L{}; int rc;
    {
        const int npasses0 = (B + zk->max_inflight - 1) / zk->max_inflight, per0 = (B + npasses0 - 1) / npasses0;
        if ((rc = lanes_ensure(zk, per0, lane0 >= 0 ? lane0 : 0, lane0 >= 0 ? 1 : std::min(zk->nlanes, npasses0)))) return rc;
    }
    hipStream_t st0 = (lane0 >= 0 && !zk->serial_streams && B <= zk->max_inflight) ? ctx->lanes[lane0].st : ctx->stream;
    zkc_zkey::CallSlot& CS = zk->call[cs];
    if (CS.pending) return zkc_fail(ctx, ZKC_ERR_BAD_ARG, "prove_batch_begin: this call slot has a call in flight (finish it first)");
    if (CS.cap < (size_t)B) {
        if (CS.d_rs) { ZKC_HIP_CHECK(ctx, hipFree(CS.d_rs)); ZKC_HIP_CHECK(ctx, hipFree(CS.d_proofs)); ZKC_HIP_CHECK(ctx, hipHostFree(CS.h_out)); ZKC_HIP_CHECK(ctx, hipHostFree(CS.h_rs)); ZKC_HIP_CHECK(ctx, hipFree(CS.d_xyzz)); ZKC_HIP_CHECK(ctx, hipHostFree(CS.h_xyzz));
                       CS.d_rs = CS.d_proofs = CS.h_out = CS.h_rs = CS.d_xyzz = CS.h_xyzz = nullptr; CS.cap = 0; }
        const size_t want = std::max<size_t>((size_t)B, std::max<size_t>(256, std::min<size_t>(2 * CS.cap, 4096)));
        ZKC_HIP_CHECK(ctx, hipMalloc((void**)&CS.d_rs, 64 * want)); ZKC_HIP_CHECK(ctx, hipMalloc((void**)&CS.d_proofs, 256 * want));
        ZKC_HIP_CHECK(ctx, hipHostMalloc((void**)&CS.h_out, (256 + 32 * (size_t)zk->nPub) * want)); ZKC_HIP_CHECK(ctx, hipHostMalloc((void**)&CS.h_rs, 64 * want));
        ZKC_HIP_CHECK(ctx, hipMalloc((void**)&CS.d_xyzz, 512 * want)); ZKC_HIP_CHECK(ctx, hipHostMalloc((void**)&CS.h_xyzz, 512 * want)); CS.cap = want;
    }
    static const unsigned ev_host_flags = hipEventDisableTiming;
    for (int l = 0; l < zk->nlanes; l++) if (!CS.ev_done[l]) ZKC_HIP_CHECK(ctx, hipEventCreateWithFlags(&CS.ev_done[l], ev_host_flags));
    CS.as_xyzz.assign((size_t)B, 0); CS.lanes_used = 0;
    if (wait_first) ZKC_HIP_CHECK(ctx, hipStreamWaitEvent(st0, wait_first, 0));
    uint8_t* const h_pub = CS.h_out + 256ull * CS.cap;
    if (rs != CS.h_rs_copy.data()) CS.h_rs_copy.assign(rs, rs + 64 * (size_t)B);
    memcpy(CS.h_rs, rs, 64 * (size_t)B);
    ZKC_HIP_CHECK(ctx, hipMemcpyAsync(CS.d_rs, CS.h_rs, 64 * (size_t)B, hipMemcpyHostToDevice, st0));
    uint32_t* tmpl = nullptr;
    if (can_fold) {
        L = WitnessLayout::make(zk->nLevels);
        if ((rc = fold_prepare(zk))) return rc;
        tmpl = zkc_get_template(ctx, zk->nLevels); if (!tmpl) return ZKC_ERR_HIP;
        const size_t nflags = (size_t)B * 2 * L.n;
        if (CS.flags_cap < nflags) {
            if (CS.d_flags) { ZKC_HIP_CHECK(ctx, hipFree(CS.d_flags)); ZKC_HIP_CHECK(ctx, hipHostFree(CS.h_flags)); CS.d_flags = CS.h_flags = nullptr; CS.flags_cap = 0; }
            const size_t want = std::max(nflags, (size_t)256 * 2 * L.n);
            ZKC_HIP_CHECK(ctx, hipMalloc((void**)&CS.d_flags, want * 4)); ZKC_HIP_CHECK(ctx, hipHostMalloc((void**)&CS.h_flags, want * 4)); CS.flags_cap = want;
        }
    }
    CS.early_n = 0; CS.arg_wtns = d_wtns; CS.arg_nw = nWitness; CS.arg_publics = want_publics; CS.arg_lane0 = lane0; CS.arg_inputs = d_inputs != nullptr; CS.arg_wait = nullptr;
    const size_t ecap = MSM_MAX_JOBS / 4;
    const bool early_wanted = !no_early && can_fold && B <= zk->max_inflight && (B <= 2 ? zk->d_fb4 != nullptr : sw::on<sw::ZKC_EARLY_LAYOUT>());
    if (early_wanted && !CS.h_early) { ZKC_HIP_CHECK(ctx, hipHostMalloc((void**)&CS.h_early, (ecap + ecap * 2 * 256) * 4)); CS.early_cap = ecap; }
    if (early_wanted && host_depths) {
        bool ok = true; for (int i = 0; i < 2 * B; i++) ok = ok && host_depths[i] < (uint8_t)L.n && L.n <= 255;
        if (ok) { CS.early_n = B; CS.early_depth.assign(host_depths, host_depths + 2 * (size_t)B); }
    } else if (early_wanted && d_inputs) {
        if (!zk->d_depths) { ZKC_HIP_CHECK(ctx, hipMalloc((void**)&zk->d_depths, 2 * ecap * 4)); ZKC_HIP_CHECK(ctx, hipHostMalloc((void**)&zk->h_depths, 2 * ecap * 4)); }
        uint32_t* hd = zk->h_depths;
        if (wait_first) ZKC_HIP_CHECK(ctx, hipStreamWaitEvent(ctx->stream2, wait_first, 0));
        hipLaunchKernelGGL(zkc_input_depths, dim3(B, 2), dim3(64), 0, ctx->stream2, (const uint32_t*)d_inputs, L.nInputs, L.n, zk->d_depths);
        ZKC_HIP_CHECK(ctx, hipGetLastError());
        ZKC_HIP_CHECK(ctx, hipMemcpyAsync(hd, zk->d_depths, 8 * (size_t)B, hipMemcpyDeviceToHost, ctx->stream2));
        ZKC_HIP_CHECK(ctx, hipStreamSynchronize(ctx->stream2));
        bool ok = true; for (int i = 0; i < 2 * B; i++) ok = ok && hd[i] < (uint32_t)L.n;
        if (ok) { CS.early_n = B; CS.early_depth.resize(2 * (size_t)B); for (int i = 0; i < 2 * B; i++) CS.early_depth[i] = (uint8_t)hd[i]; }
    }
    const int npasses = (B + zk->max_inflight - 1) / zk->max_inflight;
    const int per_pass = (B + npasses - 1) / npasses;
    while ((int)CS.ev_chunk.size() < npasses) { hipEvent_t e; ZKC_HIP_CHECK(ctx, hipEventCreateWithFlags(&e, ev_host_flags)); CS.ev_chunk.push_back(e); }
    int32_t* d_status3 = nullptr;
    if (d_inputs) {
        if ((rc = zkc_ensure(ctx, (void**)&CS.d_status3, &CS.status3_cap, std::max<size_t>((size_t)B, 256) * 3 * sizeof(int32_t)))) return rc;
        d_status3 = CS.d_status3;
    }
    const int wgroup = (int)sw::value<sw::ZKC_WITNESS_GROUP>(8);
    for (int c = 0; c < npasses; c++) {
        const int p0 = c * per_pass, nb = std::min(per_pass, B - p0);
        uint32_t* wc = (uint32_t*)d_wtns + (size_t)p0 * nv * 8;
        if (d_inputs && (c % wgroup == 0 || c == 1)) {
            const int glast = c == 0 ? 1 : std::min(((c / wgroup) + 1) * wgroup, npasses);
            const int g0 = p0, gn = std::min((glast - c) * per_pass, B - g0);
            if (gn > 0 && (rc = zkc_witness_chunk_async(ctx, zk->nLevels, (const uint8_t*)d_inputs + (size_t)g0 * L.nInputs * 32, gn, wc, d_status3 + 3 * (size_t)g0, d_status + g0, st0))) return rc;
        }
        if (can_fold) {
            uint32_t* fl = CS.d_flags + (size_t)p0 * 2 * L.n;
            hipLaunchKernelGGL(zkc_fold_check, dim3(L.n, 2, nb), dim3(64), 0, st0, L, (const uint32_t*)wc, tmpl, fl, nb);
            ZKC_HIP_CHECK(ctx, hipGetLastError());
            ZKC_HIP_CHECK(ctx, hipMemcpyAsync(CS.h_flags + (size_t)p0 * 2 * L.n, fl, (size_t)nb * 2 * L.n * 4, hipMemcpyDeviceToHost, st0));
        }
        if (CS.early_n) {
            if (d_status) ZKC_HIP_CHECK(ctx, hipMemcpyAsync(CS.h_early, d_status, 4 * (size_t)B, hipMemcpyDeviceToHost, st0));
            else memset(CS.h_early, 0, 4 * (size_t)B);
            ZKC_HIP_CHECK(ctx, hipMemcpyAsync(CS.h_early + CS.early_cap, CS.d_flags + (size_t)p0 * 2 * L.n, (size_t)nb * 2 * L.n * 4, hipMemcpyDeviceToHost, st0));
        }
        ZKC_HIP_CHECK(ctx, hipEventRecord(CS.ev_chunk[c], st0));
    }
    const bool trace_host = sw::on<sw::ZKC_TRACE_HOST>();
    auto now_ms = [] { timespec t; clock_gettime(CLOCK_MONOTONIC, &t); return t.tv_sec * 1e3 + t.tv_nsec * 1e-6; };
    const double t_begin = now_ms(); double tr[6] = {0};
    int pass = 0, done_on_st_lane = -1;
    const bool one_lane = lane0 >= 0 || zk->nlanes == 1;
    for (int p0 = 0; p0 < B; p0 += per_pass, pass++) {
        const int nb = std::min(per_pass, B - p0);
        const int li = lane0 >= 0 ? lane0 : pass % zk->nlanes; CS.lanes_used |= 1u << li;
        zkc_lane& LN = ctx->lanes[li]; const LaneSt LS = lane_st(zk, LN); const int slot = LN.npass & 1;
        tr[0] = now_ms();
        const bool early = CS.early_n > 0;
        if (!early) ZKC_HIP_CHECK(ctx, zkc_wait_event(CS.ev_chunk[pass]));
        tr[1] = now_ms();
        ZKC_HIP_CHECK(ctx, hipStreamWaitEvent(LS.st, CS.ev_chunk[pass], 0)); ZKC_HIP_CHECK(ctx, hipStreamWaitEvent(LS.st2, CS.ev_chunk[pass], 0));
        hipStream_t st = LS.st, st2 = LS.st2, fin = LS.fin;
        const uint32_t* w0 = (const uint32_t*)d_wtns + (size_t)p0 * nv * 8;
        uint8_t dcq[MSM_MAX_JOBS / 4], dsq[MSM_MAX_JOBS / 4]; bool fold = can_fold;
        if (early) for (int q = 0; q < nb; q++) { dcq[q] = CS.early_depth[2 * q]; dsq[q] = CS.early_depth[2 * q + 1]; }
        else for (int q = 0; q < nb && fold; q++) for (int t = 0; t < 2; t++) {
            const uint32_t* f = CS.h_flags + ((size_t)(p0 + q) * 2 + t) * L.n;
            if (f[L.n - 1]) { fold = false; break; }
            int D = 0; for (int g = 0; g < L.n - 1; g++) if (f[g]) D = g + 1;
            (t == 0 ? dcq : dsq)[q] = (uint8_t)D;
        }
        static thread_local zkc_zkey::Fold::VMap vms[MSM_MAX_JOBS / 4];
        if (fold) for (int q = 0; q < nb; q++) if ((rc = fold_vmap(zk, dcq[q], dsq[q], &vms[q]))) return rc;
        const bool nofold_lists = sw::on<sw::ZKC_NOFOLD_LISTS>();
        if (!fold && nofold_lists) {
            zkc_zkey::Fold::VMap nf; if ((rc = nofold_vmap(zk, &nf))) return rc;
            for (int q = 0; q < nb; q++) vms[q] = nf;
        }
        const bool listed = fold || (nofold_lists && vms[0].d != nullptr);
        if (LN.npass >= 2) { ZKC_HIP_CHECK(ctx, hipStreamWaitEvent(st, LN.ev_fin[slot], 0)); ZKC_HIP_CHECK(ctx, hipStreamWaitEvent(st2, LN.ev_fin[slot], 0)); }
        LN.npass++;
        const bool mv_prefetch = !sw::on<sw::ZKC_MATVEC_INLINE>() && one_lane;
        const bool mv_done = mv_prefetch && pass > 0;
        if (mv_done) ZKC_HIP_CHECK(ctx, hipStreamWaitEvent(st, LN.ev_mv, 0));
        if ((rc = h_evals_dev(zk, LN, st, w0, nb, !mv_done))) return rc;
        ZKC_HIP_CHECK(ctx, hipEventRecord(LN.ev_ntt, st));
        tr[2] = now_ms();
        static thread_local MsmJobList j1, j2;
        const uint32_t vwb_env = (uint32_t)sw::value<sw::ZKC_VW_BIG>(0), vws_env = (uint32_t)sw::value<sw::ZKC_VW_SMALL>(0);
        const uint32_t vws = nb <= 4 ? 64u : vws_env ? vws_env : nb < 32 ? 256u : 2048u, vwb = nb <= 4 ? 256u : vwb_env ? vwb_env : nb < 32 ? 1024u : 4096u;
        size_t lone_entries = 0; for (int q = 0; q < nb; q++) lone_entries += (size_t)msm_nw(MSM_C_G2_LONE) * (listed ? vms[q].nB : nv);
        const size_t deep_wires = (size_t)sw::value<sw::ZKC_DEEP_WIRES>(16000);
        size_t live_wires = 0; for (int q = 0; q < nb; q++) live_wires += listed ? (size_t)vms[q].nA + vms[q].nB + vms[q].nC : 2 * (size_t)nv + nc;
        const bool deep = zk->c_deep != 0 && nb > 2 && live_wires >= 3 * deep_wires * (size_t)nb;
        const int cw = deep ? zk->c_deep : zk->c_sec;
        const uint32_t oA = deep ? zk->offA_deep : zk->offA, oB1 = deep ? zk->offB1_deep : zk->offB1, oC = deep ? zk->offC_deep : zk->offC;
        const int c2 = (nb <= 2 && zk->d_g2_29_lone && lone_entries <= LN.w2.max_entries) ? MSM_C_G2_LONE : cw;
        const uint32_t vwg2_env = (uint32_t)sw::value<sw::ZKC_VW_G2>(0);
        j1.clear(vws, vwb, MSM_MAX_VW_G1); j2.clear(c2 == MSM_C_G2_LONE ? 128u : (vwg2_env && nb >= 32) ? vwg2_env : vws, 1024, MSM_MAX_VW_PER_JOB);
        for (int q = 0; q < nb; q++) j1.add(LN.d_p + 8 * (size_t)n * q, nullptr, n, zk->offH, n, 0, zk->c_h);
        size_t tree_entries = 0; for (int q = 0; q < nb; q++) tree_entries += (size_t)msm_nw(zk->c_h) * n + (size_t)msm_nw(zk->c_sec) * (listed ? 2 * (size_t)vms[q].nA + 2 * (size_t)vms[q].nB + vms[q].nC : 4 * (size_t)nv + nc);
        const bool tree = zk->d_fb4 != nullptr && nb <= 2 && 6 * nb <= LN.w1.max_jobs && tree_entries <= LN.w1.max_entries && (size_t)nb * (5 * msm_half(zk->c_sec) + msm_half(zk->c_h)) <= LN.w1.max_buckets;
        BlindArgs ba{}; ba.rs = CS.d_rs + 64 * (size_t)p0; ba.nv = nv;
        for (int q = 0; q < nb; q++) {
            const uint32_t* w = w0 + (size_t)q * nv * 8;
            uint32_t* bs = tree ? LN.d_bs + (size_t)q * 2 * nv * 8 : nullptr;
            if (tree) { ba.w[q] = w; ba.out[q] = bs; }
            if (listed) {
                const zkc_zkey::Fold::VMap& vm = vms[q];
                j1.add(w, vm.d + vm.offA, vm.nA, oA, nv, 0, cw);
                j1.add(w, vm.d + vm.offB, vm.nB, oB1, nv, 0, cw);
                j1.add(w, vm.d + vm.offC, vm.nC, oC, nc, (int32_t)np + 1, cw);
                if (tree) { j1.add(bs, vm.d + vm.offA, vm.nA, oA, nv, 0, cw); j1.add(bs + 8ull * nv, vm.d + vm.offB, vm.nB, oB1, nv, 0, cw); }
                j2.add(w, vm.d + vm.offB, vm.nB, 0, nv, 0, c2);
                if (tree) { ba.mapA[q] = vm.d + vm.offA; ba.nA[q] = vm.nA; ba.mapB[q] = vm.d + vm.offB; ba.nB[q] = vm.nB; }
            } else {
                j1.add(w, nullptr, nv, oA, nv, 0, cw);
                j1.add(w, nullptr, nv, oB1, nv, 0, cw);
                j1.add(w + 8ull * (np + 1), nullptr, nc, oC, nc, 0, cw);
                if (tree) { j1.add(bs, nullptr, nv, oA, nv, 0, cw); j1.add(bs + 8ull * nv, nullptr, nv, oB1, nv, 0, cw); }
                j2.add(w, nullptr, nv, 0, nv, 0, c2);
                if (tree) { ba.mapA[q] = ba.mapB[q] = nullptr; ba.nA[q] = ba.nB[q] = nv; }
            }
        }
        if (tree && (rc = blind_scalars_launch(ctx, st, ba, nb))) return rc;
        FinalizeArgs fa{};
        fa.r1 = (const G1XYZZ*)LN.w1.results + (size_t)slot * LN.w1.max_jobs; fa.r2 = (const G2XYZZ*)LN.w2.results + (size_t)slot * LN.w2.max_jobs;
        fa.foldA = zk->fold.d_foldA; fa.foldB1 = zk->fold.d_foldB1; fa.foldC = zk->fold.d_foldC; fa.foldB2 = zk->fold.d_foldB2; fa.fold_n = can_fold ? L.n : 0;
        for (int q = 0; q < nb; q++) { fa.dc[q] = fold ? dcq[q] : (uint8_t)255; fa.ds[q] = fold ? dsq[q] : (uint8_t)255; }
        fa.tblDelta1 = zk->d_tblDelta1; fa.tblAlpha1 = zk->d_tblAlpha1; fa.tblBeta1 = zk->d_tblBeta1; fa.tblDelta2 = zk->d_tblDelta2;
        fa.alpha1 = zk->alpha1; fa.beta2 = zk->beta2; fa.rs = CS.d_rs + 64 * (size_t)p0; fa.out = CS.d_proofs + 256 * (size_t)p0; fa.scratch = LN.d_fin;
        fa.per = tree ? 5 : 3; fa.fb4 = zk->d_fb4; fa.fb4g2 = zk->d_fb4g2; fa.out_xyzz = CS.d_xyzz + 512 * (size_t)p0;
        const bool g2_early = !sw::on<sw::ZKC_G2_LATE>();
        const bool g2_hold_env = sw::on<sw::ZKC_G2_ACC_HOLD>(), g2_early_env = sw::on<sw::ZKC_G2_ACC_EARLY>();
        const bool g2_acc_with_sort = g2_hold_env || ((nb < 32 || !one_lane) && !g2_early_env);
        if (g2_early) {
            if ((rc = msm_pass_g2(zk, LN.w2, j2, slot, false, st2, g2_acc_with_sort ? LN.ev_ntt : nullptr))) return rc;
            if (tree && (rc = finalize_tree_g2_launch(ctx, st2, fa, nb))) return rc;
            ZKC_HIP_CHECK(ctx, hipEventRecord(LN.ev_msm2, st2));
        }
        tr[3] = now_ms();
        ZKC_HIP_CHECK(ctx, hipStreamWaitEvent(st, LN.ev_red, 0));
        const bool red_split = sw::on<sw::ZKC_REDUCE_STREAM>() && !zk->serial_streams && nb >= 32;
        if ((rc = msm_pass_g1(zk, LN.w1, j1, slot, false, st, LN.ev_sorted, LN.ev_acc, (red_split && LS.red) ? LS.red : nullptr, LN.ev_red))) return rc;
        tr[4] = now_ms();
        if (!g2_early) {
            ZKC_HIP_CHECK(ctx, hipStreamWaitEvent(st2, LN.ev_sorted, 0));
            if ((rc = msm_pass_g2(zk, LN.w2, j2, slot, false, st2))) return rc;
            if (tree && (rc = finalize_tree_g2_launch(ctx, st2, fa, nb))) return rc;
            ZKC_HIP_CHECK(ctx, hipEventRecord(LN.ev_msm2, st2));
        }
        if (want_publics)
            ZKC_HIP_CHECK(ctx, hipMemcpy2DAsync(h_pub + 32ull * np * p0, 32ull * np, w0 + 8, 32ull * nv, 32ull * np, nb, hipMemcpyDeviceToHost, st));
        ZKC_HIP_CHECK(ctx, hipEventRecord(LN.ev_msm, st));
        if (mv_prefetch && p0 + per_pass < B) {
            const int p1 = p0 + per_pass, nb1 = std::min(per_pass, B - p1);
            ZKC_HIP_CHECK(ctx, hipStreamWaitEvent(fin, sw::on<sw::ZKC_MV_PREFETCH_AT_NTT>() ? LN.ev_ntt : LN.ev_sorted, 0));
            ZKC_HIP_CHECK(ctx, hipStreamWaitEvent(fin, CS.ev_chunk[pass + 1], 0));
            if ((rc = h_matvec_dev(zk, LN, (const uint32_t*)d_wtns + (size_t)p1 * nv * 8, nb1, fin))) return rc;
            ZKC_HIP_CHECK(ctx, hipEventRecord(LN.ev_mv, fin));
        }
        hipStream_t bl = ((tree || lane0 >= 0) && npasses == 1) ? st : fin;
        if (bl == fin) { ZKC_HIP_CHECK(ctx, hipStreamWaitEvent(fin, LN.ev_msm, 0)); ZKC_HIP_CHECK(ctx, hipStreamWaitEvent(fin, LN.ev_red, 0)); }
        else { if (LN.npass >= 2) ZKC_HIP_CHECK(ctx, hipStreamWaitEvent(st, LN.ev_fin[slot ^ 1], 0)); if (red_split) ZKC_HIP_CHECK(ctx, hipStreamWaitEvent(st, LN.ev_red, 0)); }
        if (!tree) ZKC_HIP_CHECK(ctx, hipStreamWaitEvent(bl, LN.ev_msm2, 0));
        if ((rc = finalize_launch(ctx, bl, fa, nb))) return rc;
        if (tree) ZKC_HIP_CHECK(ctx, hipStreamWaitEvent(bl, LN.ev_msm2, 0));
        if (tree) { ZKC_HIP_CHECK(ctx, hipMemcpyAsync(CS.h_xyzz + 512ull * p0, CS.d_xyzz + 512 * (size_t)p0, 512ull * nb, hipMemcpyDeviceToHost, bl)); for (int q = 0; q < nb; q++) CS.as_xyzz[p0 + q] = 1; }
        else ZKC_HIP_CHECK(ctx, hipMemcpyAsync(CS.h_out + 256ull * p0, CS.d_proofs + 256 * (size_t)p0, 256ull * nb, hipMemcpyDeviceToHost, bl));
        ZKC_HIP_CHECK(ctx, hipEventRecord(LN.ev_fin[slot], bl));
        if (bl == st) done_on_st_lane = li;
        tr[5] = now_ms();
        if (trace_host) fprintf(stderr, "[zkc host] pass %2d: start %8.2f | chunk wait %6.2f | h_evals %6.2f | g2 pass %6.2f | g1 pass %6.2f | blinding %6.2f ms\n", pass, tr[0] - t_begin,
                                tr[1] - tr[0], tr[2] - tr[1], tr[3] - tr[2], tr[4] - tr[3], tr[5] - tr[4]);
    }
    for (int l = 0; l < zk->nlanes; l++) if (CS.lanes_used >> l & 1) { const LaneSt ls = lane_st(zk, ctx->lanes[l]); ZKC_HIP_CHECK(ctx, hipEventRecord(CS.ev_done[l], done_on_st_lane == l ? ls.st : ls.fin)); }
    CS.B = B; CS.pending = true;
    return ZKC_OK;
}
static std::atomic<unsigned long long> g_early_retries{0};
extern "C" unsigned long long zkc_debug_early_retries(void) { return g_early_retries.load(); }
int zkc::prove_batch_finish(zkc_zkey* zk, int cs, uint8_t* proofs, uint8_t* publics) {
    if (!zk || !proofs || cs < 0 || cs >= CALL_SLOTS) return zkc_fail(zk ? zk->ctx : nullptr, ZKC_ERR_BAD_ARG, "prove_batch_finish: bad argument");
    zkc_zkey::CallSlot& CS = zk->call[cs];
    if (!CS.pending) return zkc_fail(zk->ctx, ZKC_ERR_BAD_ARG, "prove_batch_finish: no call in flight on this slot");
    hipError_t e = hipSuccess;
    for (int l = 0; l < zk->nlanes && e == hipSuccess; l++) if (CS.lanes_used >> l & 1) e = zkc_wait_event(CS.ev_done[l], CS.B <= 2 ? 6000u : 0u);
    CS.pending = false;
    if (e != hipSuccess) { ZKC_LOCK(zk->ctx); return zkc_fail(zk->ctx, ZKC_ERR_HIP, std::string("prove_batch_finish: ") + hipGetErrorString(e)); }
    if (CS.early_n) {
        const WitnessLayout L = WitnessLayout::make(zk->nLevels);
        for (int q = 0; q < CS.early_n; q++) {
            if ((int32_t)CS.h_early[q] != ZKC_W_OK) continue;
            for (int t = 0; t < 2; t++) {
                const uint32_t* f = CS.h_early + CS.early_cap + ((size_t)q * 2 + t) * L.n;
                int D = 0; for (int g = 0; g < L.n - 1; g++) if (f[g]) D = g + 1;
                if (f[L.n - 1] || D > (int)CS.early_depth[2 * q + t]) {
                    if (!CS.arg_inputs) { g_early_retries++; int rc = prove_batch_begin(zk, cs, CS.arg_wtns, CS.arg_nw, CS.B, CS.h_rs_copy.data(), CS.arg_publics, nullptr, nullptr, CS.arg_lane0, nullptr, nullptr, true); if (rc) return rc; return prove_batch_finish(zk, cs, proofs, publics); }
                    ZKC_LOCK(zk->ctx); return zkc_fail(zk->ctx, ZKC_ERR_GENERIC, "prove_batch_finish: the witness does not fold at the depth its inputs gave (internal error)");
                }
            }
        }
    }
    memcpy(proofs, CS.h_out, 256ull * CS.B);
    for (int q = 0; q < CS.B; q++) if (CS.as_xyzz[q]) {
        const uint8_t* x = CS.h_xyzz + 512 * (size_t)q; uint8_t* o = proofs + 256 * (size_t)q;
        G1XYZZ a, c; G2XYZZ b; memcpy(&a, x, 128); memcpy(&b, x + 128, 256); memcpy(&c, x + 384, 128);
        g1_to_std(o, xyzz_to_affine_gcd(a)); g2_to_std(o + 64, xyzz_to_affine_gcd(b)); g1_to_std(o + 192, xyzz_to_affine_gcd(c));
    }
    if (publics) memcpy(publics, CS.h_out + 256ull * CS.cap, 32ull * zk->nPub * CS.B);
    return ZKC_OK;
}
static int prove_batch_impl(zkc_zkey* zk, const void* d_wtns, uint32_t nWitness, int B, const uint8_t* rs, uint8_t* proofs, uint8_t* publics,
                            const void* d_inputs, int32_t* d_status) {
    if (!zk || !proofs) return zkc_fail(zk ? zk->ctx : nullptr, ZKC_ERR_BAD_ARG, "zkc_prove_batch_dev: bad argument");
// ... 43 lines not shown
```

zk-franchise-proof-circuit_amd/csrc/zkc_prover.h:

```cpp
#pragma once
#include <cstring>
#include "zkc_internal.h"
#include "zkc_curve.h"

namespace zkc {
constexpr int MSM_C_BIG = 17, MSM_C_SMALL = 12;
constexpr int MSM_C_G2_LONE = 8;
inline long long first_unreduced_wire(const void* w, size_t count) {
    const uint8_t* p = (const uint8_t*)w;
    for (size_t i = 0; i < count; i++) {
        uint32_t t[8]; memcpy(t, p + 32 * i, 32);
        if (t[7] >= FrParams::p[7] && !fp_std_lt_p<FrParams>(t)) return (long long)i;
    }
    return -1;
}
inline std::string unreduced_wire_msg(long long wire) { return "Witness value at wire " + std::to_string(wire) + " is not below the field order r"; }
inline int msm_c_for(size_t W) { return W < 12000 ? 12 : W < 22000 ? 13 : W < 90000 ? 15 : W < 180000 ? 16 : 17; }
constexpr int msm_nw(int c) { return (254 + c) / c; }
constexpr int msm_half(int c) { return 1 << (c - 1); }
constexpr int MSM_VW_MIN = 64, MSM_MAX_VW_PER_JOB = 64;
constexpr int MSM_MAX_VW_G1 = 256;
constexpr int MSM_SEG_MIN = 16;
#ifndef ZKC_MSM_SEG
#define ZKC_MSM_SEG 128
// ... 92 lines not shown
    uint32_t *vals = nullptr, *vals2 = nullptr;
    uint32_t *hist = nullptr, *bin_start = nullptr;
    uint32_t *tilecnt = nullptr; size_t max_tilecnt = 0;
    uint32_t *off = nullptr, *bcnt = nullptr;
    uint32_t *segcnt = nullptr, *segoff = nullptr, *seg2bucket = nullptr, *heavy = nullptr;
    uint32_t *seglen = nullptr, *perm = nullptr;
    uint32_t *scan_blk = nullptr, *lencnt = nullptr; size_t max_lencnt = 0;
    void *partial = nullptr;
    void *wres = nullptr;
    void *results = nullptr;
    void *h_results = nullptr;
    MsmJobList* d_jobs = nullptr;
    MsmWindow* d_windows = nullptr; size_t max_buckets = 0, max_bins = 0, max_windows = 0;
    uint16_t* d_tilejob = nullptr; uint16_t* h_tilejob[2] = {nullptr, nullptr}; size_t max_tiles = 0;
    MsmJobList* h_jobs[2] = {nullptr, nullptr}; MsmWindow* h_windows[2] = {nullptr, nullptr}; hipEvent_t h_ev[2] = {nullptr, nullptr}; int h_next = 0;
    size_t max_entries = 0, max_segments = 0; int max_jobs = 0; size_t xyzz_size = 0;
};
}

struct zkc_lane {
    hipStream_t st = nullptr, st2 = nullptr, fin = nullptr;
    hipStream_t red = nullptr; hipEvent_t ev_red = nullptr;
    zkc::Fr *d_abc = nullptr, *d_t = nullptr; uint32_t* d_p = nullptr;
    void* d_fin = nullptr;
    uint32_t* d_bs = nullptr;
    zkc::MsmWork w1, w2;
    size_t cap_abc = 0, cap_p = 0, cap_fin = 0, cap_bs = 0, bytes = 0; bool made = false;
    hipEvent_t ev_msm = nullptr, ev_msm2 = nullptr, ev_sorted = nullptr, ev_ntt = nullptr, ev_mv = nullptr, ev_acc = nullptr, ev_fin[2] = {nullptr, nullptr}; int npass = 0;
};

struct zkc_zkey {
    zkc_ctx* ctx = nullptr;
    uint32_t nVars = 0, nPub = 0, n = 0, logn = 0, nCoeffs = 0;
    int nLevels = -1;
    zkc::G1Affine alpha1, beta1, delta1;
    zkc::G2Affine beta2, gamma2, delta2;
    std::vector<zkc::G1Affine> ic;
    uint32_t *d_perm = nullptr, *d_rowlen = nullptr, *d_jdptr = nullptr, *d_col = nullptr; zkc::Fr* d_val = nullptr; uint32_t nlong = 0;
    uint32_t n_unit_coeffs = 0;
    zkc::Fr *d_tw_fwd = nullptr, *d_tw_inv = nullptr, *d_coset = nullptr;
    zkc::Fr *d_coset_br = nullptr;
    uint32_t *d_tw_fwd29 = nullptr, *d_tw_inv29 = nullptr;
    zkc::G1Affine* d_g1 = nullptr; zkc::G2Affine* d_g2 = nullptr;
    uint32_t* d_g2_29 = nullptr;
    uint32_t* d_g2_29_lone = nullptr;
    uint32_t offA = 0, offB1 = 0, offC = 0, offH = 0;
    int c_deep = 0; uint32_t offA_deep = 0, offB1_deep = 0, offC_deep = 0; uint32_t* d_g2_29_deep = nullptr;
    int c_h = zkc::MSM_C_BIG;
    int c_sec = zkc::MSM_C_SMALL;
    int max_inflight = 0;
    uint8_t sha256[32] = {0};
    size_t bytes_tables = 0;
    uint8_t fingerprint[32] = {0};
    int nlanes = 1; bool serial_streams = false;
    zkc::G1Affine *d_tblDelta1 = nullptr, *d_tblAlpha1 = nullptr, *d_tblBeta1 = nullptr; zkc::G2Affine* d_tblDelta2 = nullptr;
    uint32_t *d_depths = nullptr, *h_depths = nullptr; size_t depths_cap = 0;
    zkc::G1XYZZ* d_fb4 = nullptr; zkc::G2XYZZ* d_fb4g2 = nullptr; int fb4_bases = 0;
    struct CallSlot {
        uint8_t *d_rs = nullptr, *d_proofs = nullptr; size_t cap = 0;
        uint8_t* h_out = nullptr;
        uint8_t* h_rs = nullptr;
        uint8_t *d_xyzz = nullptr, *h_xyzz = nullptr; std::vector<uint8_t> as_xyzz;
        hipEvent_t ev_done[zkc::MAX_LANES] = {};
        std::vector<hipEvent_t> ev_chunk;
        uint32_t lanes_used = 0;
        int B = 0; bool pending = false;
        uint32_t *d_flags = nullptr, *h_flags = nullptr; size_t flags_cap = 0;
        int32_t* d_status3 = nullptr; size_t status3_cap = 0;
        int early_n = 0; std::vector<uint8_t> early_depth; uint32_t* h_early = nullptr; size_t early_cap = 0;
        const void* arg_wtns = nullptr; uint32_t arg_nw = 0; bool arg_publics = false, arg_inputs = false; int arg_lane0 = -1; hipEvent_t arg_wait = nullptr; std::vector<uint8_t> h_rs_copy;
    } call[zkc::CALL_SLOTS];
    struct Fold {
        std::vector<zkc::G1XYZZ> baseA, baseB1, baseC; std::vector<zkc::G2XYZZ> baseB2;
        std::vector<zkc::G1XYZZ> sufA[2], sufB1[2], sufC[2]; std::vector<zkc::G2XYZZ> sufB2[2];
        struct VMap { uint32_t* d = nullptr; uint32_t offA = 0, nA = 0, offB = 0, nB = 0, offC = 0, nC = 0; };
        std::map<std::pair<int, int>, VMap> vmaps;
        std::vector<uint8_t> infA, infB, infC;
        zkc::G1XYZZ *d_foldA = nullptr, *d_foldB1 = nullptr, *d_foldC = nullptr; zkc::G2XYZZ* d_foldB2 = nullptr;
        bool ready = false;
    } fold;
};

namespace zkc {
int ntt_run(zkc_ctx* ctx, hipStream_t st, const Fr* src, Fr* dst, const uint32_t* tw29, const Fr* scale, int logn, int nvec);
int ntt_make_tw29(zkc_ctx* ctx, const Fr* d_tw, uint32_t count, uint32_t** out);
int ntt_pair_run(zkc_ctx* ctx, hipStream_t st, Fr* data, const uint32_t* tw_inv29, const uint32_t* tw_fwd29, const Fr* scale_br, int logn, int nvec);
int ntt_bitrev_table(zkc_ctx* ctx, const Fr* d_src, Fr** out, int logn);
int msm_work_alloc(zkc_ctx* ctx, MsmWork& w, size_t max_entries, size_t max_buckets, int max_jobs, bool g2);
void msm_work_free(MsmWork& w);
int msm_pass_g1(zkc_zkey* zk, MsmWork& w, const MsmJobList& jl, int slot, bool to_host, hipStream_t st, hipEvent_t ev_sorted = nullptr, hipEvent_t ev_acc = nullptr,
                hipStream_t st_red = nullptr, hipEvent_t ev_red = nullptr);
int msm_pass_g2(zkc_zkey* zk, MsmWork& w, const MsmJobList& jl, int slot, bool to_host, hipStream_t st, hipEvent_t wait_before_acc = nullptr);
int msm_bucket_entries(zkc_ctx* ctx, MsmWork& w, const MsmJobList& jl, hipStream_t st, unsigned long long* d_entry_counter = nullptr);
int msm_build_segments(zkc_ctx* ctx, MsmWork& w, const MsmJobList& jl, uint32_t seg, size_t seg_bound, hipStream_t st);
int finalize_launch(zkc_ctx* ctx, hipStream_t st, const FinalizeArgs& a, int nproofs);
int finalize_tree_g2_launch(zkc_ctx* ctx, hipStream_t st, const FinalizeArgs& a, int nproofs);
int fb4_build(zkc_ctx* ctx, hipStream_t st, const G1XYZZ* d_bases, int nbases, G1XYZZ* d_out, const G2XYZZ& delta2, const G2XYZZ& beta2, const G2XYZZ& beta2_base, G2XYZZ* d_out2);
int blind_scalars_launch(zkc_ctx* ctx, hipStream_t st, const BlindArgs& a, int nproofs);
int prove_batch_begin(zkc_zkey* zk, int cs, const void* d_wtns, uint32_t nWitness, int B, const uint8_t* rs, bool want_publics, const void* d_inputs, int32_t* d_status,
                      int lane0 = -1, hipEvent_t wait_first = nullptr, const uint8_t* host_depths = nullptr, bool no_early = false);
int prove_batch_finish(zkc_zkey* zk, int cs, uint8_t* proofs, uint8_t* publics);
int prove_reserve(zkc_zkey* zk, int inflight);
int zkey_load_opts(zkc_ctx* ctx, const void* zkey_bytes, size_t len, int nlanes, int max_inflight, zkc_zkey** out);
size_t zkey_device_bytes(const zkc_zkey* zk, size_t* tables, size_t* work);
size_t finalize_scratch_bytes(int nproofs);
int msm_precompute_g1(zkc_ctx* ctx, uint32_t count, G1Affine* d_table, int c);
// ... 10 lines not shown
```

zk-franchise-proof-circuit_amd/csrc/zkc_service.hip:

```cpp
#include "zkc_prover.h"
#include "zkc_hostparse.h"
#include <algorithm>
#include <atomic>
#include <chrono>
#include <condition_variable>
#include <deque>
#include <map>
#include <memory>
#include <mutex>
#include <set>
#include <string>
#include <thread>
#include <vector>

namespace sw = zkc::sw;
int zkc_lane_streams(zkc_ctx* ctx, int l, bool with_red, zkc_ctx::LaneStreams* out);
namespace {
enum { KIND_FULLPROVE = 0, KIND_PROVE = 1 };
struct KeyImage {
    uint8_t fp[32], sha[32]; std::vector<uint8_t> bytes;
    std::set<std::pair<const void*, size_t>> confirmed;
    uint64_t last_use = 0;
    int shape_nl = -2;
};
struct Req {
    int kind; std::shared_ptr<KeyImage> img; int nLevels; const uint8_t* data; uint32_t nW; void* pin = nullptr;
    uint8_t rs[64]; uint8_t* proof; uint8_t* pub;
    zkc_done_fn done; void* user;
    bool same_class(const Req& o) const { return kind == o.kind && nLevels == o.nLevels && img.get() == o.img.get(); }
};
struct Waiter { std::mutex m; std::condition_variable cv; bool finished = false; int rc = 0; int32_t status = 0; std::string err; };
void waiter_done(void* u, int rc, int32_t status, const char* err) {
    Waiter* w = (Waiter*)u; std::lock_guard<std::mutex> g(w->m);
    w->rc = rc; w->status = status; w->err = err ? err : ""; w->finished = true; w->cv.notify_one();
}
struct HipBuf {
    void* p = nullptr; size_t sz = 0; bool host = false;
    bool ensure(size_t want) {
        if (sz >= want) return true;
        release();
        const hipError_t e = host ? hipHostMalloc(&p, want) : hipMalloc(&p, want);
        if (e != hipSuccess) { (void)hipGetLastError(); p = nullptr; return false; }
        sz = want; return true;
    }
    void release() { if (p) { if (host) (void)hipHostFree(p); else (void)hipFree(p); } p = nullptr; sz = 0; }
};
struct PinPool {
    std::mutex m; size_t total = 0, max_total = (size_t)2 << 30; std::map<size_t, std::vector<void*>> free_; std::map<void*, size_t> cls_of; std::vector<void*> chunks;
    static size_t cls(size_t bytes) { return (bytes + 262143) & ~(size_t)262143; }
    void* get(size_t bytes) {
        const size_t sl = cls(bytes);
        {
            std::lock_guard<std::mutex> g(m);
            auto& fl = free_[sl];
            if (!fl.empty()) { void* r = fl.back(); fl.pop_back(); return r; }
            if (total + 2 * sl > max_total) return nullptr;
            total += 2 * sl;
        }
        void* p = nullptr;
        if (hipHostMalloc(&p, 2 * sl, hipHostMallocPortable) != hipSuccess) { (void)hipGetLastError(); std::lock_guard<std::mutex> g(m); total -= 2 * sl; return nullptr; }
        std::lock_guard<std::mutex> g(m);
        chunks.push_back(p); cls_of[p] = sl; cls_of[(uint8_t*)p + sl] = sl; free_[sl].push_back((uint8_t*)p + sl);
        return p;
    }
    void put(void* p) { if (!p) return; std::lock_guard<std::mutex> g(m); free_[cls_of[p]].push_back(p); }
    size_t bytes() { std::lock_guard<std::mutex> g(m); return total; }
    void release() { for (void* p : chunks) (void)hipHostFree(p); chunks.clear(); cls_of.clear(); free_.clear(); total = 0; }
};
}
// ... 146 lines not shown
        if (!rc) { std::lock_guard<std::mutex> fl(d->fl_mu); zkc_service::KeySlot k; k.img = img; k.key = key; k.last_use = ++d->use_clock; d->keys.push_back(k); }
        std::lock_guard<std::mutex> g(s->mu); s->key_loads++;
        if (!rc) { d->resident.push_back(img); *out = key; }
    }
    { std::lock_guard<std::mutex> g(s->mu); if (d->loading.get() == img.get()) { d->loading.reset(); dispatch(s); } }
    return rc;
}
uint64_t now_us() { return (uint64_t)std::chrono::duration_cast<std::chrono::microseconds>(std::chrono::steady_clock::now().time_since_epoch()).count(); }
void stop_collecting(zkc_service* s, zkc_service::Worker* w) { w->collecting = nullptr; w->room = 0; if (w->dev->collector == w) w->dev->collector = nullptr; dispatch(s); }
struct CollectorGuard { zkc_service* s; zkc_service::Worker* w; ~CollectorGuard() { std::lock_guard<std::mutex> g(s->mu); if (w->dev->collector == w) stop_collecting(s, w); } };

void process(zkc_service* s, zkc_service::Worker* w, std::vector<Req*>&& first) {
    zkc_service::Dev* d = w->dev;
    CollectorGuard cguard{s, w};
    Batch b; b.reqs = std::move(first);
    const Req cls = *b.reqs[0];
    struct LoadingGuard { zkc_service* s; zkc_service::Dev* d; const KeyImage* img; ~LoadingGuard() { std::lock_guard<std::mutex> g(s->mu); if (d->loading.get() == img) d->loading.reset(); } } lguard{s, d, cls.img.get()};
    const bool full = cls.kind == KIND_FULLPROVE;
    std::string err;
    if (hipSetDevice(d->device) != hipSuccess) { (void)hipGetLastError(); return fail_all(s, b, ZKC_ERR_HIP, "hipSetDevice failed"); }
    zkc::parse::BinSections bs; zkc::parse::ZkeyHeader zh;
    if (!zkc::parse::binfile_sections(cls.img->bytes.data(), cls.img->bytes.size(), "zkey", 1, bs, err) || !zkc::parse::zkey_check(bs, zh, err, false)) return fail_all(s, b, ZKC_ERR_FORMAT, err);
    const size_t nW = zh.nVars, nPub = zh.nPub, nIn = full ? (size_t)zkc_circuit_n_inputs(cls.nLevels) : 0;
    if (full && (nIn == 0 || (size_t)zkc_circuit_n_wires(cls.nLevels) != nW)) return fail_all(s, b, ZKC_ERR_BAD_ARG, "the key is not a ZkFranchiseProofCircuit(" + std::to_string(cls.nLevels) + ") key");
    int shape_nl = cls.nLevels;
    if (!full) {
        std::lock_guard<std::mutex> g(s->img_mu);
        if (cls.img->shape_nl == -2) { cls.img->shape_nl = -1; if (nPub == 8) for (int nl = 3; nl <= 253; nl++) if ((size_t)zkc_circuit_n_wires(nl) == nW) { cls.img->shape_nl = nl; break; } }
        shape_nl = cls.img->shape_nl;
    }
    auto depths_of = [&](const Req* r, uint8_t out[2]) {
        out[0] = out[1] = 255;
        if (shape_nl < 3 || shape_nl > 253) return;
        const uint8_t* v = (const uint8_t*)(r->pin ? r->pin : r->data);
        for (int t = 0; t < 2; t++) {
            const int d = full ? last_nonzero(v + 32 * (12 + (size_t)t * (shape_nl + 1)), shape_nl + 1) : last_nonzero(v + 32 * (13 + (size_t)t * shape_nl), shape_nl);
            out[t] = d <= shape_nl ? (uint8_t)d : (uint8_t)255;
        }
    };
    auto keep_right_length = [&](std::vector<Req*>& in) {
        for (Req* r : in) { if (full || r->nW == nW) { b.reqs.push_back(r); uint8_t dd[2]; depths_of(r, dd); b.depths.push_back(dd[0]); b.depths.push_back(dd[1]); } else finish(s, r, ZKC_ERR_INVALID_WITNESS_LENGTH, 0, "Invalid witness length. Circuit: " + std::to_string(nW) + ", witness: " + std::to_string(r->nW)); }
    };
    { std::vector<Req*> in; in.swap(b.reqs); keep_right_length(in); if (b.reqs.empty()) return; }
    const size_t kind_max = full ? (size_t)s->max_batch : std::min<size_t>((size_t)s->max_batch, 128);
    w->cap = std::min(kind_max, std::max(w->cap, b.reqs.size() > 1 ? kind_max : (size_t)8));
    if (b.reqs.size() > w->cap) {
        std::lock_guard<std::mutex> g(s->mu);
        while (b.reqs.size() > w->cap) { s->q.push_front(b.reqs.back()); b.reqs.pop_back(); b.depths.pop_back(); b.depths.pop_back(); }
    }
    const size_t cap = w->cap;
    if (!w->st) {
        std::lock_guard<std::mutex> gpu(d->gpu_mu);
        if (!d->ctx && zkc_ctx_create(d->device, &d->ctx)) { d->ctx = nullptr; return fail_all(s, b, ZKC_ERR_HIP, std::string("device ") + std::to_string(d->device) + ": " + zkc_last_error(nullptr)); }
        zkc_ctx::LaneStreams ls; if (zkc_lane_streams(d->ctx, w->slot % zkc::MAX_LANES, false, &ls)) return fail_all(s, b, ZKC_ERR_HIP, zkc_last_error(d->ctx));
        w->st = ls.st;
    }
    if (!w->ev_up && hipEventCreateWithFlags(&w->ev_up, hipEventDisableTiming) != hipSuccess) { (void)hipGetLastError(); w->ev_up = nullptr; return fail_all(s, b, ZKC_ERR_HIP, "hipEventCreate failed"); }
    if ((full && (!w->h_in.ensure(cap * nIn * 32) || !w->d_in.ensure(cap * nIn * 32))) || !w->d_wtns.ensure(cap * nW * 32) || !w->d_status.ensure(cap * 4) ||
        !w->h_proofs.ensure(cap * 256) || !w->h_pubs.ensure(cap * nPub * 32 + 32) || !w->h_status.ensure(cap * 4))
        return fail_all(s, b, ZKC_ERR_HIP, "out of memory for the service's staging buffers on device " + std::to_string(d->device));
    const uint64_t t_a = now_us();
    if (!stage(w, b, 0, nIn, nW, err)) { (void)hipGetLastError(); return fail_all(s, b, ZKC_ERR_HIP, err); }
    int rc = ZKC_OK; zkc_zkey* zk = nullptr;
    uint64_t t_b = now_us(), t_c = 0, t_d = 0, t_e = 0;
    {
        const uint64_t t0 = now_us(); int quiet = 0; bool first = true;
        for (;;) {
            size_t want; { std::lock_guard<std::mutex> g(s->mu); want = std::min(cap, batch_target(s, d, b.reqs.size())); }
            if (b.reqs.size() >= want) break;
            bool busy; { std::lock_guard<std::mutex> fl(d->fl_mu); busy = d->calls_in_flight() > 0; }
            const uint64_t waited = now_us() - t0;
            if (busy ? (quiet >= 2 || waited >= s->busy_wait_us) : (quiet >= 3 || waited >= 3000)) break;
            std::vector<Req*> more;
            {
                std::unique_lock<std::mutex> lk(s->mu);
                more = grab(s, w, want - b.reqs.size(), &cls);
                if (more.empty()) {
                    if (!busy && first && b.reqs.size() == 1) break;
                    w->collecting = &cls; w->room = want - b.reqs.size(); w->wake = false;
                    w->cv.wait_for(lk, std::chrono::microseconds(busy ? 100 : 50), [&] { return w->wake || s->stop; });
                    w->wake = false; w->collecting = nullptr; w->room = 0;
                    if (s->stop) break;
                    want = std::min(cap, batch_target(s, d, b.reqs.size()));
                    if (want > b.reqs.size()) more = grab(s, w, want - b.reqs.size(), &cls);
                }
            }
            first = false;
            if (more.empty()) { quiet++; continue; }
            quiet = 0;
            const size_t from = b.reqs.size();
            keep_right_length(more);
            if (!stage(w, b, from, nIn, nW, err)) { (void)hipGetLastError(); return fail_all(s, b, ZKC_ERR_HIP, err); }
        }
        std::lock_guard<std::mutex> g(s->mu); stop_collecting(s, w);
    }
    if (hipEventRecord(w->ev_up, w->st) != hipSuccess) { (void)hipGetLastError(); return fail_all(s, b, ZKC_ERR_HIP, "hipEventRecord failed"); }
    {
        std::lock_guard<std::mutex> gpu(d->gpu_mu);
        t_c = now_us();
        const int B = (int)b.reqs.size();
        { std::string why; if ((rc = ensure_key(s, d, cls.img, &zk, why))) return fail_all(s, b, rc, why); }
        if (full && zk->nLevels != cls.nLevels) return fail_all(s, b, ZKC_ERR_BAD_ARG, "the key is not a ZkFranchiseProofCircuit(" + std::to_string(cls.nLevels) + ") key");
        b.rs.resize((size_t)B * 64);
        for (int i = 0; i < B; i++) memcpy(b.rs.data() + 64 * (size_t)i, b.reqs[i]->rs, 64);
        t_d = now_us();
        rc = zkc::prove_batch_begin(zk, w->slot, w->d_wtns.p, (uint32_t)nW, B, b.rs.data(), true, full ? w->d_in.p : nullptr, full ? (int32_t*)w->d_status.p : nullptr, w->slot % zk->nlanes, w->ev_up,
                                     b.depths.size() == 2 * (size_t)B ? b.depths.data() : nullptr);
// ... 20 lines not shown
        if (st == ZKC_W_OK) { memcpy(r->proof, (const uint8_t*)w->h_proofs.p + 256 * i, 256); if (r->pub) memcpy(r->pub, (const uint8_t*)w->h_pubs.p + nPub * 32 * i, nPub * 32); }
        const char* why = st == ZKC_W_OK ? "" : zkc_witness_status_text(r->nLevels, st);
        finish(s, r, st == ZKC_W_OK ? ZKC_OK : ZKC_ERR_WITNESS, st, why ? why : "a circuit assert failed (see status)");
    }
    { std::lock_guard<std::mutex> g(s->mu); s->us_finish += now_us() - t_e; }
}
void worker_main(zkc_service* s, zkc_service::Worker* w) {
    std::unique_lock<std::mutex> lk(s->mu);
    for (;;) {
        std::vector<Req*> batch;
        while (!s->stop && !w->warm && (w->dev->collector || (batch = grab(s, w, std::min<size_t>((size_t)s->max_batch, batch_target(s, w->dev, 0)))).empty())) {
            w->idle = true; w->cv.wait(lk, [&] { return w->wake || s->stop; }); w->wake = false; w->idle = false;
        }
        if (!s->stop && w->warm) {
            std::shared_ptr<KeyImage> img = std::move(w->warm); w->warm.reset();
            lk.unlock();
            if (hipSetDevice(w->dev->device) == hipSuccess) { std::lock_guard<std::mutex> gpu(w->dev->gpu_mu); std::string why; zkc_zkey* k = nullptr; (void)ensure_key(s, w->dev, img, &k, why); }
            else { (void)hipGetLastError(); std::lock_guard<std::mutex> g(s->mu); if (w->dev->loading.get() == img.get()) w->dev->loading.reset(); }
            lk.lock();
            dispatch(s);
            continue;
        }
        if (s->stop) { for (Req* r : batch) s->q.push_front(r); break; }
        w->dev->collector = w;
        dispatch(s);
        lk.unlock();
        process(s, w, std::move(batch));
        lk.lock();
    }
    lk.unlock();
    (void)hipSetDevice(w->dev->device);
    for (HipBuf* hb : {&w->h_in, &w->h_wtns, &w->d_in, &w->d_wtns, &w->d_status, &w->h_proofs, &w->h_pubs, &w->h_status}) hb->release();
    if (w->ev_up) (void)hipEventDestroy(w->ev_up);
}
int service_fail(int code, const std::string& msg) { g_service_err = msg; return code; }
bool parse_device_list(const char* e, std::vector<int>& out) {
    int count = 0;
    if (hipGetDeviceCount(&count) != hipSuccess) { (void)hipGetLastError(); count = 0; }
    if (!e || !*e || !strcmp(e, "all")) { for (int i = 0; i < count; i++) out.push_back(i); return !out.empty(); }
    for (const char* p = e; *p;) { char* end; const long v = strtol(p, &end, 10); if (end == p || v < 0) return false; out.push_back((int)v); p = *end == ',' ? end + 1 : end; if (*end && *end != ',') return false; }
    return !out.empty();
}
}

extern "C" const char* zkc_service_last_error(void) { return g_service_err.c_str(); }
extern "C" int zkc_service_create(const int* hip_devices, int n, zkc_service** out) {
    if (!out || n < 0 || n > 64 || (n > 0 && !hip_devices)) return service_fail(ZKC_ERR_BAD_ARG, "zkc_service_create: bad argument");
    std::vector<int> devs(hip_devices, hip_devices + n);
    if (n == 0 && !parse_device_list(sw::text<sw::ZKC_DEVICE>(), devs)) return service_fail(ZKC_ERR_HIP, "zkc_service_create: no GPU visible (or $ZKC_DEVICE is not a list of device numbers)");
    zkc_service* s = new zkc_service();
    s->max_batch = (int)sw::value<sw::ZKC_SERVICE_MAX_BATCH>(s->max_batch);
    s->spill = (int)sw::value<sw::ZKC_SERVICE_SPILL>(s->spill);
    s->keys_per_dev = (int)sw::value<sw::ZKC_SERVICE_KEYS>(s->keys_per_dev);
    s->workers_per_dev = (int)sw::value<sw::ZKC_SERVICE_WORKERS>(s->workers_per_dev);
    s->pass = (int)sw::value<sw::ZKC_SERVICE_PASS>(s->pass);
    s->busy_wait_us = (uint64_t)sw::value<sw::ZKC_SERVICE_BUSY_WAIT_US>((long long)s->busy_wait_us);
    s->min_batch = (int)sw::value<sw::ZKC_SERVICE_MIN_BATCH>(s->min_batch);
    for (int dv : devs) { s->devs.emplace_back(new zkc_service::Dev()); s->devs.back()->device = dv; }
    int idx = 0;
    for (auto& d : s->devs) for (int k = 0; k < s->workers_per_dev; k++) { s->workers.emplace_back(new zkc_service::Worker()); s->workers.back()->dev = d.get(); s->workers.back()->index = idx++; s->workers.back()->slot = k; }
    for (auto& w : s->workers) w->th = std::thread(worker_main, s, w.get());
    *out = s; return ZKC_OK;
}
extern "C" void zkc_service_destroy(zkc_service* s) {
    if (!s) return;
    { std::lock_guard<std::mutex> g(s->mu); s->stop = true; for (auto& w : s->workers) w->cv.notify_all(); }
    for (auto& w : s->workers) if (w->th.joinable()) w->th.join();
    for (Req* r : s->q) finish(s, r, ZKC_ERR_GENERIC, 0, "the proving service was shut down");
    s->q.clear();
    for (auto& d : s->devs) { (void)hipSetDevice(d->device); for (auto& k : d->keys) if (k.key) zkc_zkey_free(k.key); if (d->ctx) zkc_ctx_destroy(d->ctx); }
    s->pin.release();
    delete s;
}
extern "C" zkc_service* zkc_service_default(void) {
    static std::mutex mu; static zkc_service* svc = nullptr;
    static std::string why;
    std::lock_guard<std::mutex> g(mu);
    if (!svc && zkc_service_create(nullptr, 0, &svc)) { svc = nullptr; why = g_service_err; }
    if (!svc) g_service_err = why;
    return svc;
}
static std::shared_ptr<KeyImage> image_of(zkc_service* s, const void* zkey, size_t zkey_len, std::string& why) {
    uint8_t fp[32];
    if (zkc_zkey_fingerprint(zkey, zkey_len, fp)) { why = "not a zkey file"; return nullptr; }
    std::lock_guard<std::mutex> g(s->img_mu);
    const std::pair<const void*, size_t> ident(zkey, zkey_len);
    bool sha_known = false; uint8_t sha[32];
    for (auto& im : s->images) {
        if (memcmp(im->fp, fp, 32) || im->bytes.size() != zkey_len) continue;
        if (!im->confirmed.count(ident)) {
            if (!sha_known) { zkc::parse::sha256(zkey, zkey_len, sha); sha_known = true; }
            if (memcmp(sha, im->sha, 32)) continue;
            if (im->confirmed.size() > 256) im->confirmed.clear();
            im->confirmed.insert(ident);
        }
        im->last_use = ++s->img_clock;
        return im;
    }
    auto im = std::make_shared<KeyImage>();
    memcpy(im->fp, fp, 32);
    if (!sha_known) zkc::parse::sha256(zkey, zkey_len, sha);
    memcpy(im->sha, sha, 32);
    im->bytes.assign((const uint8_t*)zkey, (const uint8_t*)zkey + zkey_len);
    im->confirmed.insert(ident); im->last_use = ++s->img_clock;
    const size_t keep = std::max<size_t>(8, (size_t)s->keys_per_dev * s->devs.size());
    while (s->images.size() >= keep) {
// ... 91 lines not shown
```

zk-franchise-proof-circuit_amd/csrc/zkc_switches.h:

```cpp
#pragma once
#include <climits>
#include <cstdlib>
#include <optional>

namespace zkc { namespace sw {

enum Kind { SET, OFF_IF_ZERO, ON_IF_ONE, NUMBER, NUMBER_LONG, NUMBER_U64, TEXT };
enum When { PROCESS, LIVE };
constexpr long long ANY = LLONG_MIN;

#define ZKC_SWITCHES(X)                                                                                                                                                   \
                                                                                                                                            \
    X(ZKC_DEVICE,               TEXT,        ANY, ANY,   LIVE,    "service creation: the GPUs of the default proving service: \"2\", \"0,1,2,3\", \"all\"; unset: every visible device") \
    X(ZKC_INFLIGHT,             NUMBER,      1,   128,   LIVE,    "key load: proofs per pipeline pass (census key 64, any other 96, fewer for a large circuit); at most MSM_MAX_JOBS / 4") \
    X(ZKC_LANES,                NUMBER,      1,   4,     LIVE,    "key load: pipeline lanes the passes of a batch call rotate over (census key MAX_LANES = 4, any other 1)")      \
    X(ZKC_DEEP_TABLES,          NUMBER,      ANY, ANY,   LIVE,    "key load: 0 leaves out the second section tables that passes of deep voters take, 2 builds them for a census key of any size (default 1)") \
    X(ZKC_G2_LONE_TABLE,        OFF_IF_ZERO, ANY, ANY,   LIVE,    "key load: =0 skips the 8-bit-window G2 table of the lone-proof path")                                          \
    X(ZKC_BLIND_TREE,           OFF_IF_ZERO, ANY, ANY,   LIVE,    "key load: =0 gives a key whose passes of one or two proofs take the general blinding kernels")                 \
    X(ZKC_SERVICE_WORKERS,      NUMBER,      1,   4,     LIVE,    "service creation: workers (= lanes of a service key) per GPU (4); at most MAX_LANES")                          \
    X(ZKC_SERVICE_PASS,         NUMBER,      1,   128,   LIVE,    "service creation: proofs per pass of a service key (64); at most MSM_MAX_JOBS / 4")                            \
    X(ZKC_SERVICE_KEYS,         NUMBER,      1,   64,    LIVE,    "service creation: keys kept resident per GPU (4)")                                                             \
    X(ZKC_SERVICE_MAX_BATCH,    NUMBER,      1,   4096,  LIVE,    "service creation: requests one worker takes per call (256)")                                                   \
    X(ZKC_SERVICE_MIN_BATCH,    NUMBER,      1,   ANY,   LIVE,    "service creation: requests a collecting worker waits for before it goes (16)")                                 \
    X(ZKC_SERVICE_SPILL,        NUMBER,      1,   ANY,   LIVE,    "service creation: queue length at which a cold GPU is brought up (32)")                                        \
    X(ZKC_SERVICE_BUSY_WAIT_US, NUMBER,      0,   ANY,   LIVE,    "service creation: microseconds a collecting worker waits for more requests (300)")                             \
    X(ZKC_SERVICE_RESERVE,      OFF_IF_ZERO, ANY, ANY,   PROCESS, "=0: a service key load does not reserve a full pass of work space on every lane; the lanes grow on demand")    \
    X(ZKC_DEVICE_BLOCKING_SYNC, ON_IF_ONE,   ANY, ANY,   LIVE,    "context creation: =1 asks HIP for blocking waits on the device (hipDeviceScheduleBlockingSync)")               \
    X(ZKC_SPIN_WAIT,            SET,         ANY, ANY,   PROCESS, "set (any value, 0 included): host waits use hipEventSynchronize instead of polling with short sleeps")         \
    X(ZKC_VERIFY_BATCH_GPU,     NUMBER,      ANY, ANY,   LIVE,    "per verify call: 0 keeps the Miller loops of zkc_verify_batch on the host, positive forces the GPU, negative or unset: GPU from 128 proofs") \
    X(ZKC_NO_SHA_NI,            SET,         ANY, ANY,   PROCESS, "set (any value, 0 included): portable SHA-256 instead of the CPU's SHA extensions")                            \
                                                                                                                              \
    X(ZKC_NO_FOLD,              SET,         ANY, ANY,   LIVE,    "key load: set (any value, 0 included): no constant folding of the voter-independent witness part for this key") \
    X(ZKC_SERIAL_STREAMS,       SET,         ANY, ANY,   LIVE,    "key load: set (any value, 0 included): every stage of this key's passes on the context's one stream (isolated stage times)") \
    X(ZKC_C_SECTIONS,           NUMBER,      8,   17,    LIVE,    "key load: window bits of the witness sections (census key 12, any other by its wire count); at most MSM_C_BIG") \
    X(ZKC_C_H,                  NUMBER,      8,   17,    LIVE,    "key load: window bits of the H section (census key 17, any other by its domain size); at most MSM_C_BIG")      \
    X(ZKC_C_DEEP,               NUMBER,      13,  17,    LIVE,    "key load: window bits of the second section tables (by the wire count); at most MSM_C_BIG")                    \
    X(ZKC_DEEP_WIRES,           NUMBER_LONG, ANY, ANY,   PROCESS, "live wires per section and proof from which a pass takes the second section tables (16000)")                   \
    X(ZKC_WITNESS_GROUP,        NUMBER,      1,   ANY,   PROCESS, "passes whose voters share one witness launch in a batch call (8)")                                             \
    X(ZKC_VW_BIG,               NUMBER,      ANY, ANY,   PROCESS, "buckets per reduction wave of the H jobs in passes of more than four proofs (0 or unset: 4096, 1024 below 32 proofs)") \
    X(ZKC_VW_SMALL,             NUMBER,      ANY, ANY,   PROCESS, "the same for the witness sections (0 or unset: 2048, 256 below 32 proofs)")                                    \
    X(ZKC_VW_G2,                NUMBER,      ANY, ANY,   PROCESS, "the same for the G2 jobs of passes of 32 proofs and more (0 or unset: as the witness sections)")              \
    X(ZKC_G2_ACC,               NUMBER,      ANY, ANY,   PROCESS, "form of the G2 accumulation: 0 registers hold the next row, 1 / 2 LDS-DMA prefetch at one / two waves per SIMD (0)") \
    X(ZKC_G2_BUCKET_WAVE,       OFF_IF_ZERO, ANY, ANY,   PROCESS, "=0: small G2 passes keep lane-per-segment accumulation instead of half a wave per bucket")                     \
    X(ZKC_G2_LATE,              SET,         ANY, ANY,   PROCESS, "set (any value, 0 included): the G2 MSM of a pass starts after the G1 sort instead of with the pass")          \
    X(ZKC_G2_ACC_HOLD,          SET,         ANY, ANY,   PROCESS, "set (any value, 0 included): the G2 accumulation always waits for the G1 stream to leave its transforms")      \
    X(ZKC_G2_ACC_EARLY,         SET,         ANY, ANY,   PROCESS, "set (any value, 0 included): the G2 accumulation never waits for them (ZKC_G2_ACC_HOLD wins)")                 \
    X(ZKC_ACC_CHAIN,            OFF_IF_ZERO, ANY, ANY,   PROCESS, "=0: the G1 accumulations of a context's lanes are not chained one behind the other")                           \
    X(ZKC_REDUCE_STREAM,        ON_IF_ONE,   ANY, ANY,   PROCESS, "=1: the bucket reduction of a full pass runs on a stream of its own (the lanes then get that stream)")         \
    X(ZKC_MATVEC_UNITS,         OFF_IF_ZERO, ANY, ANY,   PROCESS, "=0: buildABC multiplies by its +-1 coefficients instead of adding the wire")                                   \
    X(ZKC_MATVEC_INLINE,        SET,         ANY, ANY,   PROCESS, "set (any value, 0 included): buildABC of the next pass is not prefetched on the blinding stream")              \
    X(ZKC_MV_PREFETCH_AT_NTT,   ON_IF_ONE,   ANY, ANY,   PROCESS, "=1: that prefetch starts beside the pass' bucketing instead of beside its accumulation")                       \
    X(ZKC_EARLY_LAYOUT,         OFF_IF_ZERO, ANY, ANY,   PROCESS, "=0: one-pass calls of more than two voters wait for their fold flags instead of reading the depths off the inputs") \
    X(ZKC_NOFOLD_LISTS,         OFF_IF_ZERO, ANY, ANY,   PROCESS, "=0: unfolded passes keep the wires whose bases are at infinity")                                               \
    X(ZKC_NTT_SEPARATE,         SET,         ANY, ANY,   PROCESS, "set (any value, 0 included): two self-contained transforms instead of the fused pair")                         \
    X(ZKC_NTT_RADIX,            NUMBER,      ANY, ANY,   PROCESS, "below 4: the head transform kernel runs one stage at a time instead of two (4)")                               \
    X(ZKC_FINALIZE_WAVES,       SET,         ANY, ANY,   PROCESS, "set (any value, 0 included): the one-wave-per-task blinding kernel for every pass")                            \
    X(ZKC_VERIFY_CHUNK,         NUMBER,      2,   16384, LIVE,    "per verify call: pairs per round of Miller-loop kernels (16384)")                                              \
    X(ZKC_SMT_WAVE_MAX,         NUMBER_U64,  ANY, ANY,   LIVE,    "per check call: census proof batches up to this size take the wave-per-proof form (64; 0: never)")            \
    X(ZKC_TRACE_HOST,           SET,         ANY, ANY,   PROCESS, "set (any value, 0 included): prints where the enqueueing thread spends its time, per pass")                    \
    X(ZKC_VERIFY_TRACE,         SET,         ANY, ANY,   LIVE,    "per verify call: set (any value, 0 included): prints the stage times of zkc_verify_batch")                     \
    X(ZKC_DEBUG_SYNC,           SET,         ANY, ANY,   PROCESS, "set (any value, 0 included): synchronises after and logs every MSM launch; read when the library is loaded")   \
                                                                                                                                                \
    X(ZKC_TEST_FAIL_ALLOC,      NUMBER,      ANY, ANY,   LIVE,    "lane growth: the work-space allocation for this many proofs in flight or more fails")                          \
    X(ZKC_TEST_FAIL_KEY_LOADS,  NUMBER,      ANY, ANY,   LIVE,    "service key load: fails as out of memory while the device holds this many keys or more")

enum Id {
#define X(name, kind, lo, hi, when, doc) name,
    ZKC_SWITCHES(X)
#undef X
    COUNT
};
struct Row { const char* name; Kind kind; long long lo, hi; When when; const char* doc; };
inline constexpr Row rows[COUNT] = {
#define X(name, kind, lo, hi, when, doc) {#name, kind, lo, (hi) == ANY ? LLONG_MAX : (hi), when, doc},
    ZKC_SWITCHES(X)
#undef X
};

struct Raw { bool set; long long num; const char* str; };
inline Raw read(const Row& r) {
    const char* e = getenv(r.name);
    if (!e) return {false, 0, nullptr};
    const long long v = r.kind == NUMBER_U64 ? (long long)strtoull(e, nullptr, 10) : r.kind == NUMBER_LONG ? (long long)atol(e) : (long long)atoi(e);
    return {true, v < r.lo ? r.lo : v > r.hi ? r.hi : v, e};
}
template <Id I> inline Raw get() {
    if constexpr (rows[I].when == PROCESS) { static const Raw cached = read(rows[I]); return cached; }
    else return read(rows[I]);
}
constexpr bool is_number(Kind k) { return k == NUMBER || k == NUMBER_LONG || k == NUMBER_U64; }

template <Id I> inline bool on() {
    static_assert(rows[I].kind == SET || rows[I].kind == OFF_IF_ZERO || rows[I].kind == ON_IF_ONE, "not an on/off switch");
    const Raw r = get<I>();
    return rows[I].kind == SET ? r.set : rows[I].kind == OFF_IF_ZERO ? !(r.set && r.num == 0) : (r.set && r.num == 1);
}
template <Id I> inline std::optional<long long> given() {
    static_assert(is_number(rows[I].kind), "not a number");
    const Raw r = get<I>();
    return r.set ? std::optional<long long>(r.num) : std::nullopt;
}
template <Id I> inline long long value(long long dflt) { return given<I>().value_or(dflt); }
template <Id I> inline const char* text() {
    static_assert(rows[I].kind == TEXT && rows[I].when == LIVE, "not a live text switch");
    return get<I>().str;
}

}}
```

Before: 2963.

## Add narrow stream plan that caps busy streams to hardware queue count

Adds a stream plan that reads GPU_MAX_HW_QUEUES (4 when unset) and, below 16 queues, switches to a narrow plan. Under that plan the context skips its side streams, a census key uses one lane instead of four, and each lane gets only as many streams as the queues allow. Helper kernels fall back to the main stream, and service workers are capped at half the queue count. The aim is to stop many HIP streams from being multiplexed onto a few hardware queues, which can add false dependencies and scheduling overhead. The cost is less lane-level overlap between passes. A query API is also added to report which streams were used.

```diff
diff --git a/include/zkcensus.h b/include/zkcensus.h
--- a/include/zkcensus.h
+++ b/include/zkcensus.h
@@ -45,6 +45,7 @@
 void zkc_zkey_free(zkc_zkey* zk);
 int  zkc_zkey_info(const zkc_zkey* zk, uint32_t* nVars, uint32_t* nPublic, uint32_t* domainSize);
 int  zkc_zkey_pass_info(const zkc_zkey* zk, int* pass_size, int* lanes);
+int  zkc_stream_plan_info(zkc_ctx* ctx, const zkc_zkey* zk, int reset, int out[4]);
 int  zkc_zkey_header_info(const void* zkey_bytes, size_t len, uint32_t* nVars, uint32_t* nPublic, uint32_t* domainSize);
 int  zkc_zkey_sha256(const zkc_zkey* zk, uint8_t out[32]);
 int  zkc_zkey_fingerprint(const void* zkey_bytes, size_t len, uint8_t out[32]);
diff --git a/zk-franchise-proof-circuit_amd/__init__.py b/zk-franchise-proof-circuit_amd/__init__.py
--- a/zk-franchise-proof-circuit_amd/__init__.py
+++ b/zk-franchise-proof-circuit_amd/__init__.py
@@ -75,6 +75,11 @@
         ps, ln = ctypes.c_int(), ctypes.c_int()
         self._lib.zkc_zkey_pass_info(h, ctypes.byref(ps), ctypes.byref(ln))
         self.pass_size, self.lanes = ps.value, ln.value
+
+    def stream_plan_info(self, reset=True):
+        out = (ctypes.c_int * 4)()
+        self.ctx._check(self._lib.zkc_stream_plan_info(self.ctx._h, self._h, 1 if reset else 0, out))
+        return tuple(out)
 
     def close(self):
         if getattr(self, '_h', None):
diff --git a/zk-franchise-proof-circuit_amd/_native.py b/zk-franchise-proof-circuit_amd/_native.py
--- a/zk-franchise-proof-circuit_amd/_native.py
+++ b/zk-franchise-proof-circuit_amd/_native.py
@@ -36,6 +36,7 @@
     L.zkc_zkey_free.argtypes = [vp]; L.zkc_zkey_free.restype = None
     L.zkc_zkey_info.argtypes = [vp, u32p, u32p, u32p]
     L.zkc_zkey_pass_info.argtypes = [vp, ctypes.POINTER(ctypes.c_int), ctypes.POINTER(ctypes.c_int)]
+    L.zkc_stream_plan_info.argtypes = [vp, vp, ctypes.c_int, ctypes.POINTER(ctypes.c_int)]
     L.zkc_witness_status_text.argtypes = [ctypes.c_int, ctypes.c_int32]; L.zkc_witness_status_text.restype = ctypes.c_char_p
     L.zkc_prove.argtypes = [vp, ctypes.c_char_p, ctypes.c_uint32, u8p, u8p, ctypes.c_char_p, ctypes.c_char_p]
     L.zkc_prove_dev.argtypes = [vp, vp, ctypes.c_uint32, u8p, u8p, ctypes.c_char_p, ctypes.c_char_p]
diff --git a/zk-franchise-proof-circuit_amd/csrc/zkc_api.hip b/zk-franchise-proof-circuit_amd/csrc/zkc_api.hip
--- a/zk-franchise-proof-circuit_amd/csrc/zkc_api.hip
+++ b/zk-franchise-proof-circuit_amd/csrc/zkc_api.hip
@@ -81,7 +81,7 @@
     if (!ctx || cat < 0 || cat >= ZKC_PROF_NCAT) return ZKC_ERR_BAD_ARG;
     ZKC_LOCK(ctx);
     ZKC_HIP_CHECK(ctx, hipSetDevice(ctx->device));
-    ZKC_HIP_CHECK(ctx, hipStreamSynchronize(ctx->stream)); ZKC_HIP_CHECK(ctx, hipStreamSynchronize(ctx->stream2)); ZKC_HIP_CHECK(ctx, hipStreamSynchronize(ctx->fin_stream));
+    ZKC_HIP_CHECK(ctx, hipStreamSynchronize(ctx->stream)); if (ctx->stream2) ZKC_HIP_CHECK(ctx, hipStreamSynchronize(ctx->stream2)); if (ctx->fin_stream) ZKC_HIP_CHECK(ctx, hipStreamSynchronize(ctx->fin_stream));
     for (auto& r : ctx->prof.pending) {
         float ms = 0; (void)hipEventElapsedTime(&ms, r.a, r.b); ctx->prof.ms[r.cat] += ms;
         ctx->prof.free_events.push_back(r.a); ctx->prof.free_events.push_back(r.b);
@@ -143,8 +143,11 @@
     if ((e = hipSetDevice(device)) != hipSuccess) return fail(e, "hipSetDevice");
     { if (sw::on<sw::ZKC_DEVICE_BLOCKING_SYNC>() && hipSetDeviceFlags(hipDeviceScheduleBlockingSync) != hipSuccess) (void)hipGetLastError(); }
     if ((e = hipStreamCreateWithFlags(&ctx->stream, hipStreamNonBlocking)) != hipSuccess) return fail(e, "hipStreamCreate");
-    if ((e = hipStreamCreateWithFlags(&ctx->stream2, hipStreamNonBlocking)) != hipSuccess) return fail(e, "hipStreamCreate(2)");
-    if ((e = hipStreamCreateWithFlags(&ctx->fin_stream, hipStreamNonBlocking)) != hipSuccess) return fail(e, "hipStreamCreate(fin)");
+    ctx->narrow = sw::narrow_streams();
+    if (!ctx->narrow) {
+        if ((e = hipStreamCreateWithFlags(&ctx->stream2, hipStreamNonBlocking)) != hipSuccess) return fail(e, "hipStreamCreate(2)");
+        if ((e = hipStreamCreateWithFlags(&ctx->fin_stream, hipStreamNonBlocking)) != hipSuccess) return fail(e, "hipStreamCreate(fin)");
+    }
     std::vector<Fr> all; size_t off[12]; int k = 0;
     off[k++] = all.size(); conv_consts(all, ZKC_POSEIDON_C3); off[k++] = all.size(); conv_consts(all, ZKC_POSEIDON_S3);
     off[k++] = all.size(); conv_consts(all, ZKC_POSEIDON_M3); off[k++] = all.size(); conv_consts(all, ZKC_POSEIDON_P3);
@@ -215,12 +218,23 @@
     if (ctx->stream) (void)hipStreamDestroy(ctx->stream);
     delete ctx;
 }
-int zkc_lane_streams(zkc_ctx* ctx, int l, bool with_red, zkc_ctx::LaneStreams* out) {
-    if (!ctx || l < 0 || l >= 4 || !out) return ZKC_ERR_BAD_ARG;
+int zkc_side_streams(zkc_ctx* ctx) {
+    for (hipStream_t* q : {&ctx->stream2, &ctx->fin_stream}) if (!*q) ZKC_HIP_CHECK(ctx, hipStreamCreateWithFlags(q, hipStreamNonBlocking));
+    return ZKC_OK;
+}
+extern "C" int zkc_stream_plan_info(zkc_ctx* ctx, const zkc_zkey* zk, int reset, int* out) {
+    if (!ctx || !out) return ZKC_ERR_BAD_ARG;
+    ZKC_LOCK(ctx);
+    out[0] = ctx->narrow ? 2 : 1; { int ps = 0, ln = 0; if (zk) (void)zkc_zkey_pass_info(zk, &ps, &ln); out[1] = ln; } out[2] = (int)ctx->used_streams.size(); out[3] = sw::hw_queues();
+    if (reset) ctx->used_streams.clear();
+    return ZKC_OK;
+}
+int zkc_lane_streams(zkc_ctx* ctx, int l, bool with_red, zkc_ctx::LaneStreams* out, int nstreams) {
+    if (!ctx || l < 0 || l >= 4 || !out || nstreams < 1 || nstreams > 3) return ZKC_ERR_BAD_ARG;
     static std::mutex mu; static std::map<int, std::array<zkc_ctx::LaneStreams, 4>> by_device;
     std::lock_guard<std::mutex> g(mu);
     zkc_ctx::LaneStreams& ls = by_device[ctx->device][l];
-    for (hipStream_t* q : {&ls.st, &ls.st2, &ls.fin}) if (!*q) ZKC_HIP_CHECK(ctx, hipStreamCreateWithFlags(q, hipStreamNonBlocking));
+    { int k = 0; for (hipStream_t* q : {&ls.st, &ls.st2, &ls.fin}) if (k++ < nstreams && !*q) ZKC_HIP_CHECK(ctx, hipStreamCreateWithFlags(q, hipStreamNonBlocking)); }
     if (with_red && !ls.red) ZKC_HIP_CHECK(ctx, hipStreamCreateWithFlags(&ls.red, hipStreamNonBlocking));
     ctx->lane_streams[l] = ls; *out = ls; return ZKC_OK;
 }
diff --git a/zk-franchise-proof-circuit_amd/csrc/zkc_internal.h b/zk-franchise-proof-circuit_amd/csrc/zkc_internal.h
--- a/zk-franchise-proof-circuit_amd/csrc/zkc_internal.h
+++ b/zk-franchise-proof-circuit_amd/csrc/zkc_internal.h
@@ -27,6 +27,9 @@
     hipStream_t stream = nullptr;
     hipStream_t stream2 = nullptr;
     hipStream_t fin_stream = nullptr;
+    bool narrow = false;
+    std::vector<hipStream_t> used_streams;
+    void used(hipStream_t q) { for (hipStream_t u : used_streams) if (u == q) return; used_streams.push_back(q); }
     struct LaneStreams { hipStream_t st = nullptr, st2 = nullptr, fin = nullptr, red = nullptr; } lane_streams[4];
     struct zkc_lane* lanes = nullptr;
     hipEvent_t ev_acc_chain = nullptr; bool acc_chain_armed = false;
@@ -55,6 +58,7 @@
 };
 
 int zkc_fail(zkc_ctx* ctx, int code, const std::string& msg);
+int zkc_side_streams(zkc_ctx* ctx);
 hipError_t zkc_wait_event(hipEvent_t ev, unsigned spin_us = 0);
 hipError_t zkc_wait_stream(hipStream_t st, hipEvent_t scratch_ev);
 int zkc_ensure(zkc_ctx* ctx, void** p, size_t* cur, size_t need);
diff --git a/zk-franchise-proof-circuit_amd/csrc/zkc_pairing_dev.hip b/zk-franchise-proof-circuit_amd/csrc/zkc_pairing_dev.hip
--- a/zk-franchise-proof-circuit_amd/csrc/zkc_pairing_dev.hip
+++ b/zk-franchise-proof-circuit_amd/csrc/zkc_pairing_dev.hip
@@ -108,12 +108,13 @@
 uint32_t verify_chunk() { return (uint32_t)sw::value<sw::ZKC_VERIFY_CHUNK>(16384); }
 static uint32_t n_lines(const MillerConsts& C) { return 66 + (uint32_t)__builtin_popcountll(C.pos | C.neg); }
 uint32_t verify_n_lines() { return n_lines(miller_consts()); }
-void miller_join(zkc_ctx* ctx) { (void)hipStreamSynchronize(ctx->stream2); (void)hipStreamSynchronize(ctx->fin_stream); }
+void miller_join(zkc_ctx* ctx) { if (ctx->stream2) (void)hipStreamSynchronize(ctx->stream2); if (ctx->fin_stream) (void)hipStreamSynchronize(ctx->fin_stream); }
 
 int miller_membership_begin(zkc_ctx* ctx, const G2Affine* h_Q, uint32_t N) {
     const MillerConsts C = miller_consts();
     const uint32_t cap = std::min(N, verify_chunk());
     void* q; int rc;
+    if ((rc = zkc_side_streams(ctx))) return rc;
     if ((rc = zkc_vws(ctx, zkc_ctx::VWS_Q, (size_t)N * sizeof(G2Affine), &q))) return rc;
     G2Affine* d_Q = (G2Affine*)q;
     if ((rc = zkc_vws(ctx, zkc_ctx::VWS_BAD, sizeof(int), &q))) return rc;
diff --git a/zk-franchise-proof-circuit_amd/csrc/zkc_prove.hip b/zk-franchise-proof-circuit_amd/csrc/zkc_prove.hip
--- a/zk-franchise-proof-circuit_amd/csrc/zkc_prove.hip
+++ b/zk-franchise-proof-circuit_amd/csrc/zkc_prove.hip
@@ -42,7 +42,7 @@
 }
 
 uint32_t* zkc_get_template(zkc_ctx* ctx, int nLevels);
-int zkc_lane_streams(zkc_ctx* ctx, int l, bool with_red, zkc_ctx::LaneStreams* out);
+int zkc_lane_streams(zkc_ctx* ctx, int l, bool with_red, zkc_ctx::LaneStreams* out, int nstreams = 3);
 
 extern "C" __global__ void __launch_bounds__(64)
 zkc_fold_check(WitnessLayout L, const uint32_t* __restrict__ wtns, const uint32_t* __restrict__ tmpl, uint32_t* __restrict__ flags, int B) {
@@ -123,19 +123,27 @@
     }
     delete[] ctx->lanes; ctx->lanes = nullptr;
 }
-static int lane_init(zkc_ctx* ctx, int l) {
+static int lane_init(zkc_ctx* ctx, int l, int nstreams) {
     zkc_lane& L = ctx_lanes(ctx)[l];
+    if (ctx->narrow ? (nstreams >= 3 ? !L.fin : nstreams == 2 ? !L.st2 : !L.st) : !L.made) {
+        zkc_ctx::LaneStreams ls; int rc = zkc_lane_streams(ctx, l, !ctx->narrow && sw::on<sw::ZKC_REDUCE_STREAM>(), &ls, ctx->narrow ? nstreams : 3); if (rc) return rc;
+        L.st = ls.st; L.st2 = ls.st2; L.fin = ls.fin; L.red = ctx->narrow ? nullptr : ls.red;
+    }
     if (L.made) return ZKC_OK;
-    zkc_ctx::LaneStreams ls; int rc = zkc_lane_streams(ctx, l, sw::on<sw::ZKC_REDUCE_STREAM>(), &ls); if (rc) return rc;
-    L.st = ls.st; L.st2 = ls.st2; L.fin = ls.fin; L.red = ls.red;
     for (hipEvent_t* e : {&L.ev_msm, &L.ev_msm2, &L.ev_sorted, &L.ev_ntt, &L.ev_mv, &L.ev_acc, &L.ev_fin[0], &L.ev_fin[1], &L.ev_red}) if (!*e) ZKC_HIP_CHECK(ctx, hipEventCreateWithFlags(e, hipEventDisableTiming));
     L.made = true; return ZKC_OK;
 }
 struct LaneSt { hipStream_t st, st2, fin, red; };
-static LaneSt lane_st(const zkc_zkey* zk, const zkc_lane& L) { hipStream_t c = zk->ctx->stream; return zk->serial_streams ? LaneSt{c, c, c, c} : LaneSt{L.st, L.st2, L.fin, L.red}; }
+static LaneSt lane_st(const zkc_zkey* zk, const zkc_lane& L) {
+    hipStream_t c = zk->ctx->stream;
+    if (zk->serial_streams) return LaneSt{c, c, c, c};
+    if (zk->lane_streams == 1) return LaneSt{L.st, L.st, L.st, L.st};
+    if (zk->lane_streams == 2) return LaneSt{L.st, L.st2, L.st, L.st};
+    return LaneSt{L.st, L.st2, L.fin, zk->ctx->narrow ? L.st : L.red};
+}
 static int lane_ensure(zkc_zkey* zk, int l, int inflight) {
     zkc_ctx* ctx = zk->ctx; int rc;
-    if ((rc = lane_init(ctx, l))) return rc;
+    if ((rc = lane_init(ctx, l, zk->lane_streams))) return rc;
     zkc_lane& L = ctx->lanes[l];
     inflight = std::max(1, std::min(inflight, zk->max_inflight));
     if (lane_holds(L, lane_need(zk, inflight))) return ZKC_OK;
@@ -313,8 +321,14 @@
         const int fit = (int)std::max<size_t>(1, census_pass / std::max<size_t>(per_proof_entries, 1));
         zk->max_inflight = std::min(zk->max_inflight, fit);
     }
-    { const auto e_l = sw::given<sw::ZKC_LANES>(); zk->nlanes = opt_lanes > 0 ? std::min(opt_lanes, (int)MAX_LANES) : e_l ? (int)*e_l : zk->nLevels >= 0 ? (int)MAX_LANES : 1; }
+    const long long plan = sw::value<sw::ZKC_STREAM_PLAN>(0);
+    const bool narrow_key = plan == 2 || (plan == 0 && ctx->narrow);
+    { const auto e_l = sw::given<sw::ZKC_LANES>(); zk->nlanes = opt_lanes > 0 ? std::min(opt_lanes, (int)MAX_LANES) : e_l ? (int)*e_l : (zk->nLevels >= 0 && !narrow_key) ? (int)MAX_LANES : 1; }
     zk->serial_streams = sw::on<sw::ZKC_SERIAL_STREAMS>();
+    {
+        zk->lane_streams = narrow_key ? std::max(1, std::min(3, sw::hw_queues() / zk->nlanes)) : 3;
+        zk->front_on_lane = narrow_key && zk->nlanes * zk->lane_streams + 1 > sw::hw_queues();
+    }
     if ((rc = lanes_ensure(zk, 1, 0, 1))) return bail(rc);
     {
         FixedBase<Fq> td(zk->delta1), ta(zk->alpha1), tb(zk->beta1); FixedBase<Fq2> t2(zk->delta2);
@@ -539,7 +553,9 @@
         const int npasses0 = (B + zk->max_inflight - 1) / zk->max_inflight, per0 = (B + npasses0 - 1) / npasses0;
         if ((rc = lanes_ensure(zk, per0, lane0 >= 0 ? lane0 : 0, lane0 >= 0 ? 1 : std::min(zk->nlanes, npasses0)))) return rc;
     }
-    hipStream_t st0 = (lane0 >= 0 && !zk->serial_streams && B <= zk->max_inflight) ? ctx->lanes[lane0].st : ctx->stream;
+    hipStream_t st0 = (lane0 >= 0 && !zk->serial_streams && B <= zk->max_inflight) ? ctx->lanes[lane0].st :
+                      (zk->front_on_lane && !zk->serial_streams) ? lane_st(zk, ctx->lanes[lane0 >= 0 ? lane0 : 0]).st2 : ctx->stream;
+    ctx->used(st0);
     zkc_zkey::CallSlot& CS = zk->call[cs];
     if (CS.pending) return zkc_fail(ctx, ZKC_ERR_BAD_ARG, "prove_batch_begin: this call slot has a call in flight (finish it first)");
     if (CS.cap < (size_t)B) {
@@ -580,11 +596,13 @@
     } else if (early_wanted && d_inputs) {
         if (!zk->d_depths) { ZKC_HIP_CHECK(ctx, hipMalloc((void**)&zk->d_depths, 2 * ecap * 4)); ZKC_HIP_CHECK(ctx, hipHostMalloc((void**)&zk->h_depths, 2 * ecap * 4)); }
         uint32_t* hd = zk->h_depths;
-        if (wait_first) ZKC_HIP_CHECK(ctx, hipStreamWaitEvent(ctx->stream2, wait_first, 0));
-        hipLaunchKernelGGL(zkc_input_depths, dim3(B, 2), dim3(64), 0, ctx->stream2, (const uint32_t*)d_inputs, L.nInputs, L.n, zk->d_depths);
+        const hipStream_t sd = ctx->stream2 && !ctx->narrow ? ctx->stream2 : st0;
+        if (wait_first && sd != st0) ZKC_HIP_CHECK(ctx, hipStreamWaitEvent(sd, wait_first, 0));
+        hipLaunchKernelGGL(zkc_input_depths, dim3(B, 2), dim3(64), 0, sd, (const uint32_t*)d_inputs, L.nInputs, L.n, zk->d_depths);
         ZKC_HIP_CHECK(ctx, hipGetLastError());
-        ZKC_HIP_CHECK(ctx, hipMemcpyAsync(hd, zk->d_depths, 8 * (size_t)B, hipMemcpyDeviceToHost, ctx->stream2));
-        ZKC_HIP_CHECK(ctx, hipStreamSynchronize(ctx->stream2));
+        ZKC_HIP_CHECK(ctx, hipMemcpyAsync(hd, zk->d_depths, 8 * (size_t)B, hipMemcpyDeviceToHost, sd));
+        ZKC_HIP_CHECK(ctx, hipStreamSynchronize(sd));
+        ctx->used(sd);
         bool ok = true; for (int i = 0; i < 2 * B; i++) ok = ok && hd[i] < (uint32_t)L.n;
         if (ok) { CS.early_n = B; CS.early_depth.resize(2 * (size_t)B); for (int i = 0; i < 2 * B; i++) CS.early_depth[i] = (uint8_t)hd[i]; }
     }
@@ -633,6 +651,7 @@
         tr[1] = now_ms();
         ZKC_HIP_CHECK(ctx, hipStreamWaitEvent(LS.st, CS.ev_chunk[pass], 0)); ZKC_HIP_CHECK(ctx, hipStreamWaitEvent(LS.st2, CS.ev_chunk[pass], 0));
         hipStream_t st = LS.st, st2 = LS.st2, fin = LS.fin;
+        ctx->used(st); ctx->used(st2);
         const uint32_t* w0 = (const uint32_t*)d_wtns + (size_t)p0 * nv * 8;
         uint8_t dcq[MSM_MAX_JOBS / 4], dsq[MSM_MAX_JOBS / 4]; bool fold = can_fold;
         if (early) for (int q = 0; q < nb; q++) { dcq[q] = CS.early_depth[2 * q]; dsq[q] = CS.early_depth[2 * q + 1]; }
@@ -733,6 +752,7 @@
             ZKC_HIP_CHECK(ctx, hipEventRecord(LN.ev_mv, fin));
         }
         hipStream_t bl = ((tree || lane0 >= 0) && npasses == 1) ? st : fin;
+        ctx->used(bl); if (mv_prefetch && p0 + per_pass < B) ctx->used(fin); if (red_split && LS.red) ctx->used(LS.red);
         if (bl == fin) { ZKC_HIP_CHECK(ctx, hipStreamWaitEvent(fin, LN.ev_msm, 0)); ZKC_HIP_CHECK(ctx, hipStreamWaitEvent(fin, LN.ev_red, 0)); }
         else { if (LN.npass >= 2) ZKC_HIP_CHECK(ctx, hipStreamWaitEvent(st, LN.ev_fin[slot ^ 1], 0)); if (red_split) ZKC_HIP_CHECK(ctx, hipStreamWaitEvent(st, LN.ev_red, 0)); }
         if (!tree) ZKC_HIP_CHECK(ctx, hipStreamWaitEvent(bl, LN.ev_msm2, 0));
diff --git a/zk-franchise-proof-circuit_amd/csrc/zkc_prover.h b/zk-franchise-proof-circuit_amd/csrc/zkc_prover.h
--- a/zk-franchise-proof-circuit_amd/csrc/zkc_prover.h
+++ b/zk-franchise-proof-circuit_amd/csrc/zkc_prover.h
@@ -168,6 +168,7 @@
     uint8_t sha256[32] = {0};
     size_t bytes_tables = 0;
     uint8_t fingerprint[32] = {0};
+    int lane_streams = 3; bool front_on_lane = false;
     int nlanes = 1; bool serial_streams = false;
     zkc::G1Affine *d_tblDelta1 = nullptr, *d_tblAlpha1 = nullptr, *d_tblBeta1 = nullptr; zkc::G2Affine* d_tblDelta2 = nullptr;
     uint32_t *d_depths = nullptr, *h_depths = nullptr; size_t depths_cap = 0;
diff --git a/zk-franchise-proof-circuit_amd/csrc/zkc_service.hip b/zk-franchise-proof-circuit_amd/csrc/zkc_service.hip
--- a/zk-franchise-proof-circuit_amd/csrc/zkc_service.hip
+++ b/zk-franchise-proof-circuit_amd/csrc/zkc_service.hip
@@ -14,7 +14,7 @@
 #include <vector>
 
 namespace sw = zkc::sw;
-int zkc_lane_streams(zkc_ctx* ctx, int l, bool with_red, zkc_ctx::LaneStreams* out);
+int zkc_lane_streams(zkc_ctx* ctx, int l, bool with_red, zkc_ctx::LaneStreams* out, int nstreams = 3);
 namespace {
 enum { KIND_FULLPROVE = 0, KIND_PROVE = 1 };
 struct KeyImage {
@@ -267,7 +267,7 @@
     if (!w->st) {
         std::lock_guard<std::mutex> gpu(d->gpu_mu);
         if (!d->ctx && zkc_ctx_create(d->device, &d->ctx)) { d->ctx = nullptr; return fail_all(s, b, ZKC_ERR_HIP, std::string("device ") + std::to_string(d->device) + ": " + zkc_last_error(nullptr)); }
-        zkc_ctx::LaneStreams ls; if (zkc_lane_streams(d->ctx, w->slot % zkc::MAX_LANES, false, &ls)) return fail_all(s, b, ZKC_ERR_HIP, zkc_last_error(d->ctx));
+        zkc_ctx::LaneStreams ls; if (zkc_lane_streams(d->ctx, w->slot % zkc::MAX_LANES, false, &ls, d->ctx->narrow ? 1 : 3)) return fail_all(s, b, ZKC_ERR_HIP, zkc_last_error(d->ctx));
         w->st = ls.st;
     }
     if (!w->ev_up && hipEventCreateWithFlags(&w->ev_up, hipEventDisableTiming) != hipSuccess) { (void)hipGetLastError(); w->ev_up = nullptr; return fail_all(s, b, ZKC_ERR_HIP, "hipEventCreate failed"); }
@@ -394,6 +394,7 @@
     s->max_batch = (int)sw::value<sw::ZKC_SERVICE_MAX_BATCH>(s->max_batch);
     s->spill = (int)sw::value<sw::ZKC_SERVICE_SPILL>(s->spill);
     s->keys_per_dev = (int)sw::value<sw::ZKC_SERVICE_KEYS>(s->keys_per_dev);
+    if (sw::narrow_streams()) s->workers_per_dev = std::max(1, std::min(s->workers_per_dev, sw::hw_queues() / 2));
     s->workers_per_dev = (int)sw::value<sw::ZKC_SERVICE_WORKERS>(s->workers_per_dev);
     s->pass = (int)sw::value<sw::ZKC_SERVICE_PASS>(s->pass);
     s->busy_wait_us = (uint64_t)sw::value<sw::ZKC_SERVICE_BUSY_WAIT_US>((long long)s->busy_wait_us);
diff --git a/zk-franchise-proof-circuit_amd/csrc/zkc_switches.h b/zk-franchise-proof-circuit_amd/csrc/zkc_switches.h
--- a/zk-franchise-proof-circuit_amd/csrc/zkc_switches.h
+++ b/zk-franchise-proof-circuit_amd/csrc/zkc_switches.h
@@ -13,11 +13,12 @@
                                                                                                                                             \
     X(ZKC_DEVICE,               TEXT,        ANY, ANY,   LIVE,    "service creation: the GPUs of the default proving service: \"2\", \"0,1,2,3\", \"all\"; unset: every visible device") \
     X(ZKC_INFLIGHT,             NUMBER,      1,   128,   LIVE,    "key load: proofs per pipeline pass (census key 64, any other 96, fewer for a large circuit); at most MSM_MAX_JOBS / 4") \
-    X(ZKC_LANES,                NUMBER,      1,   4,     LIVE,    "key load: pipeline lanes the passes of a batch call rotate over (census key MAX_LANES = 4, any other 1)")      \
+    X(ZKC_LANES,                NUMBER,      1,   4,     LIVE,    "key load: pipeline lanes the passes of a batch call rotate over (census key MAX_LANES = 4 -- 1 under the narrow stream plan --, any other 1)") \
+    X(ZKC_STREAM_PLAN,          NUMBER,      0,   2,     LIVE,    "context creation, key load, service creation: 0 auto (wide from 16 hardware queues, narrow below), 1 wide: three streams per lane, 2 narrow: no more busy streams than hardware queues") \
     X(ZKC_DEEP_TABLES,          NUMBER,      ANY, ANY,   LIVE,    "key load: 0 leaves out the second section tables that passes of deep voters take, 2 builds them for a census key of any size (default 1)") \
     X(ZKC_G2_LONE_TABLE,        OFF_IF_ZERO, ANY, ANY,   LIVE,    "key load: =0 skips the 8-bit-window G2 table of the lone-proof path")                                          \
     X(ZKC_BLIND_TREE,           OFF_IF_ZERO, ANY, ANY,   LIVE,    "key load: =0 gives a key whose passes of one or two proofs take the general blinding kernels")                 \
-    X(ZKC_SERVICE_WORKERS,      NUMBER,      1,   4,     LIVE,    "service creation: workers (= lanes of a service key) per GPU (4); at most MAX_LANES")                          \
+    X(ZKC_SERVICE_WORKERS,      NUMBER,      1,   4,     LIVE,    "service creation: workers (= lanes of a service key) per GPU (4; narrow stream plan: hardware queues / 2); at most MAX_LANES") \
     X(ZKC_SERVICE_PASS,         NUMBER,      1,   128,   LIVE,    "service creation: proofs per pass of a service key (64); at most MSM_MAX_JOBS / 4")                            \
     X(ZKC_SERVICE_KEYS,         NUMBER,      1,   64,    LIVE,    "service creation: keys kept resident per GPU (4)")                                                             \
     X(ZKC_SERVICE_MAX_BATCH,    NUMBER,      1,   4096,  LIVE,    "service creation: requests one worker takes per call (256)")                                                   \
@@ -106,4 +107,13 @@
     return get<I>().str;
 }
 
+inline int hw_queues() {
+    const char* e = getenv("GPU_MAX_HW_QUEUES");
+    if (!e) return 4;
+    char* end = nullptr; const long v = strtol(e, &end, 10);
+    if (end == e) return 4;
+    return v < 1 ? 1 : v > 32 ? 32 : (int)v;
+}
+inline bool narrow_streams() { const long long p = value<ZKC_STREAM_PLAN>(0); return p == 2 || (p == 0 && hw_queues() < 16); }
+
 }}
```

After: 2991, median of 6. Within noise of the previous version (+1.0%).
